# zhenyuw16/Uni3DETR

Hardware: AMD Instinct MI355X
Metric: scenes/sec (fwd+bwd) SUN-RGB-D 20k pts, 300 queries (higher is better)
Workload: dtype bf16

## Files before the change

include/u3d_hip.h:

```cpp
#ifndef U3D_HIP_H_
#define U3D_HIP_H_

#include <stddef.h>
#include <stdint.h>

#ifdef __cplusplus
extern "C" {
#endif

typedef struct ihipStream_t* u3d_stream;

enum {
  U3D_OK = 0,
  U3D_ERR_ARG = -1,
  U3D_ERR_UNSUPPORTED = -2,
  U3D_ERR_LAUNCH = -3,
  U3D_ERR_WORKSPACE = -4
};

enum { U3D_F32 = 0, U3D_BF16 = 1 };

int32_t u3d_version(void);
const char* u3d_strerror(int32_t code);

// ... 30 lines not shown

int32_t u3d_nbr_table(const u3d_bitgrid* target, const int32_t* q_coors, const int32_t* n_dev, int32_t n_cap,
                      const int32_t ksize[3], const int32_t stride[3], const int32_t pad[3], int32_t mode,
                      int32_t* nbr, int32_t ld, u3d_stream s);

int32_t u3d_nbr_table_k3(const u3d_bitgrid* target, const int32_t* q_coors, const int32_t* n_dev, int32_t n_cap,
                         const int32_t stride[3], const int32_t pad[3], int32_t mode, int32_t* nbr, int32_t ld, u3d_stream s);

int32_t u3d_dense_nbr_table(int32_t batch, const int32_t q_dims[3], const int32_t t_dims[3], const int32_t ksize[3],
                            const int32_t stride[3], const int32_t pad[3], int32_t mode, int32_t* nbr, int32_t ld,
                            u3d_stream s);

int64_t u3d_voxelize_hard_workspace(int32_t n_total, int32_t batch, int32_t max_pts_per_scene);
int32_t u3d_voxelize_hard(const float* points, const int32_t* scene_off, int32_t batch, int32_t n_total,
                          int32_t max_pts_per_scene, int32_t nfeat, const float voxel_size[3],
                          const float pc_range[6], int32_t max_points, int32_t max_voxels,
                          float* voxels, int32_t* coors, int32_t* num_points, float* mean,
                          int32_t* voxel_off, void* workspace, int64_t workspace_bytes, u3d_stream s);
int32_t u3d_voxelize_hard_chunked(const float* points, const int32_t* scene_off, int32_t batch, int32_t n_total,
                                  int32_t max_pts_per_scene, int32_t nfeat, const float voxel_size[3],
                                  const float pc_range[6], int32_t max_points, int32_t max_voxels,
                                  float* voxels, int32_t* coors, int32_t* num_points, float* mean,
                                  int32_t* voxel_off, void* workspace, int64_t workspace_bytes, u3d_stream s);

int32_t u3d_voxelize_dynamic(const float* points, const int32_t* scene_off, int32_t batch, int32_t n_total, int32_t nfeat,
                             const float voxel_size[3], const float pc_range[6], int32_t* coors, u3d_stream s);
int32_t u3d_scatter_mean(const float* points, const int32_t* rank, int32_t n_total, int32_t nfeat, float* sums,
                         int32_t* counts, int32_t n_voxels, u3d_stream s);

int32_t u3d_spconv_fwd(const void* in, const void* w, const int32_t* nbr, int32_t ld, void* out,
                       const int32_t* n_out_dev, int32_t n_out_cap, int32_t cin, int32_t cout, int32_t kvol,
                       int32_t transpose_w, int32_t dtype, u3d_stream s);

enum { U3D_FWD_EPI_PLAIN, U3D_FWD_EPI_ADD, U3D_FWD_EPI_STATS, U3D_FWD_EPI_AFFINE, U3D_FWD_EPI_COUNT };
enum { U3D_FWD_FAM_NONE, U3D_FWD_FAM_CONV_IN, U3D_FWD_FAM_DIRECT, U3D_FWD_FAM_GLDS, U3D_FWD_FAM_REG, U3D_FWD_FAM_COUNT };
typedef struct u3d_fwd_plan_info {
  int32_t family, kernel, rows, cols, partials, rows_per_partial, takes_addend;
} u3d_fwd_plan_info;
int32_t u3d_igemm_fwd_plan(int32_t n_out_cap, int32_t cin, int32_t cout, int32_t kvol, int32_t has_nbr, int32_t nmajor, int32_t epi,
                           u3d_fwd_plan_info* info);
int32_t u3d_igemm_fwd_bf16(const void* in, const void* w, const int32_t* nbr, int32_t ld, void* out,
                           const int32_t* n_out_dev, int32_t n_out_cap, int32_t cin, int32_t cout, int32_t kvol,
                           int32_t transpose_w, const void* addend, double* stats, u3d_stream s);
int32_t u3d_linear_bf16(const void* x, const void* w, const float* bias, int32_t relu, void* out, const int32_t* m_dev,
                        int32_t m_cap, int32_t k, int32_t n, u3d_stream s);
int64_t u3d_bn_fold_job_bytes(void);
int32_t u3d_bn_fold_job_blocks(int32_t kvol, int32_t cout, int32_t cin);
int32_t u3d_bn_fold_batched(const void* jobs, int32_t njobs, int32_t total_blocks, u3d_stream s);
int32_t u3d_igemm_fwd_affine_bf16(const void* in, const void* w_folded, const int32_t* nbr, int32_t ld, const float* shift, int32_t relu,
                                  void* out, const int32_t* n_out_dev, int32_t n_out_cap, int32_t cin, int32_t cout, int32_t kvol,
                                  u3d_stream s);
int32_t u3d_igemm_fwd_split_bf16(const void* in, const void* w, const int32_t* nbr, int32_t ld, float* out, const int32_t* n_out_dev,
                                 int32_t n_out_cap, int32_t cin, int32_t cout, int32_t kvol3, double* stats, const float* addend, u3d_stream s);
int32_t u3d_igemm_direct_split_bf16(const void* in, const void* w3, const int32_t* nbr, int32_t ld, float* out, const int32_t* n_out_dev,
                                    int32_t n_out_cap, int32_t n_in_cap, int32_t cin, int32_t cout, u3d_stream s);
int32_t u3d_igemm_direct_affine_bf16(const void* in, const void* w_folded, const int32_t* nbr, int32_t ld, const float* shift,
                                     int32_t relu, const void* addend, void* out, const int32_t* n_out_dev, int32_t n_out_cap,
                                     int32_t cin, int32_t cout, u3d_stream s);
int32_t u3d_split3_weights(const float* src, int64_t sk, int64_t sa, int64_t sb, int32_t k, int32_t a, int32_t b, void* dst, u3d_stream s);
typedef struct U3dSplitRowsJobs {
  const float* src[32];
  void* dst[32];
  int32_t ld[32], rows[32], cols[32];
  int32_t first_block[33];
  int32_t njobs;
} U3dSplitRowsJobs;
int32_t u3d_split_rows_batch(const U3dSplitRowsJobs* jobs, u3d_stream s);
int32_t u3d_sum3_f32(const float* a, const float* b, const float* c, float* out, int64_t n, u3d_stream s);
int64_t u3d_split3_job_bytes(void);
int32_t u3d_split3_job_blocks(int32_t k, int32_t a, int32_t b);
int32_t u3d_split3_weights_batch(const void* jobs, int32_t njobs, int32_t total_blocks, u3d_stream s);
int32_t u3d_split_rows_f32(const float* x, const int32_t* n_dev, int32_t n_cap, int32_t c, void* dst, u3d_stream s);
int32_t u3d_subm_halo_sizes(int32_t n_cap, int64_t* tile_rows_elems, int64_t* loc_elems, int32_t* tiles);
int32_t u3d_subm_halo_build(const int32_t* nbr, int32_t ld, const int32_t* n_dev, int32_t n_cap, int32_t* tile_rows,
                            uint16_t* loc, int32_t* tile_cnt, int32_t kvol, u3d_stream s);
int32_t u3d_subm_halo_wpack(const void* w_nmajor, void* w_packed, u3d_stream s);
int32_t u3d_subm_halo_wpack_batched(const void* const* srcs_dev, void* const* dsts_dev, int32_t n, u3d_stream s);
int32_t u3d_subm_halo_conv64_bf16(const void* in, const void* w_packed, const int32_t* tile_rows, const uint16_t* loc,
                                  const int32_t* tile_cnt, const int32_t* n_dev, int32_t n_cap, int32_t krev,
                                  const void* addend, void* out, double* stats, int32_t max_slots, u3d_stream s);
int32_t u3d_subm_halo_wpack128(const void* w_nmajor, void* w_packed, int32_t kvol, u3d_stream s);
int32_t u3d_subm_halo_wpack128_batched(const void* const* srcs_dev, void* const* dsts_dev, int32_t n, int32_t kvol, u3d_stream s);
int32_t u3d_subm_halo_conv128_bf16(const void* in, const void* w_packed, const int32_t* tile_rows, const uint16_t* loc,
                                   const int32_t* tile_cnt, const int32_t* n_dev, int32_t n_cap, int32_t krev,
                                   const void* addend, void* out, double* stats, int32_t max_slots, int32_t kvol, u3d_stream s);
int32_t u3d_subm_halo_conv64_affine_bf16(const void* in, const void* w_packed, const int32_t* tile_rows, const uint16_t* loc,
                                         const int32_t* tile_cnt, const int32_t* n_dev, int32_t n_cap, const void* addend, void* out,
                                         const float* shift, int32_t relu, int32_t max_slots, u3d_stream s);
int32_t u3d_subm_halo_conv128_affine_bf16(const void* in, const void* w_packed, const int32_t* tile_rows, const uint16_t* loc,
                                          const int32_t* tile_cnt, const int32_t* n_dev, int32_t n_cap, const void* addend, void* out,
                                          const float* shift, int32_t relu, int32_t max_slots, int32_t kvol, u3d_stream s);
int64_t u3d_subm_halo_wgrad64_workspace(void);
int32_t u3d_subm_halo_wgrad64_bf16(const void* x, const void* dy, const int32_t* tile_rows, const uint16_t* loc,
                                   const int32_t* tile_cnt, const int32_t* n_dev, int32_t n_cap, float* dw, void* workspace,
                                   int64_t workspace_bytes, int32_t max_slots, u3d_stream s);
int64_t u3d_igemm_wgrad_bf16_workspace(int32_t n_out_cap, int32_t cin, int32_t cout, int32_t kvol);
int32_t u3d_igemm_wgrad_bf16(const void* in, const void* dout, const int32_t* nbr, int32_t ld, float* dw,
                             const int32_t* n_out_dev, int32_t n_out_cap, int32_t cin, int32_t cout, int32_t kvol,
                             int32_t out_layout, void* workspace, int64_t workspace_bytes, u3d_stream s);
int32_t u3d_igemm_wgrad_plan(int32_t n_out_cap, int32_t cin, int32_t cout, int32_t kvol, int32_t has_nbr, int32_t out_layout,
                             int32_t* kernel, int32_t* tile, int32_t* nsplit, int64_t* workspace);

int64_t u3d_spconv_wgrad_workspace(int32_t n_out_cap, int32_t cin, int32_t cout, int32_t kvol);
int32_t u3d_spconv_wgrad(const void* in, const void* dout, const int32_t* nbr, int32_t ld, float* dw,
                         const int32_t* n_out_dev, int32_t n_out_cap, int32_t cin, int32_t cout, int32_t kvol,
                         int32_t dtype, void* workspace, int64_t workspace_bytes, u3d_stream s);

int64_t u3d_colsum_workspace(int32_t n, int32_t c);
int32_t u3d_colsum(const void* x, int32_t n, int32_t c, int32_t dtype, float* out, void* workspace,
                   int64_t workspace_bytes, u3d_stream s);

int64_t u3d_wgrad_batched_workspace(int32_t count, int32_t n_rows, int32_t cin, int32_t cout);
int32_t u3d_wgrad_batched_bf16(const void* const* in, const void* const* dout, float* const* dw, int32_t count,
                               const int32_t* n_dev, int32_t n_rows, int32_t cin, int32_t cout, void* workspace,
                               int64_t workspace_bytes, u3d_stream s);
int64_t u3d_colsum_batched_workspace(int32_t count, int32_t n, int32_t c);
int32_t u3d_colsum_batched(const void* const* x, float* const* out, int32_t count, int32_t n, int32_t c, int32_t dtype,
                           void* workspace, int64_t workspace_bytes, u3d_stream s);

int32_t u3d_skinny_wgrad_chunks(int32_t m);
int32_t u3d_skinny_wgrad_bf16(const void* dy, const void* x, int32_t m, int32_t n, int32_t k, float* partial, u3d_stream s);
int32_t u3d_skinny_wgrad_batched(const void* const* dy, const void* const* x, float* const* partial, const int32_t* n, const int32_t* k,
                                 int32_t count, int32_t m, int32_t dy_skinny, u3d_stream s);

int64_t u3d_bn_stats_workspace(int32_t n_cap, int32_t c);
int32_t u3d_bn_stats(const void* x, const int32_t* n_dev, int32_t n_cap, int32_t c, int32_t dtype,
                     double* sums, void* workspace, int64_t workspace_bytes, u3d_stream s);
int32_t u3d_bn_finalize(const double* sums, const int32_t* n_dev, int32_t n_cap, int32_t c, float eps, float momentum,
                        float* running_mean, float* running_var, int64_t* num_batches, float* mean, float* invstd,
                        u3d_stream s);
int32_t u3d_bn_forward_stats(const void* x, const int32_t* n_dev, int32_t n_cap, int32_t c, int32_t dtype, float eps,
                             float momentum, float* running_mean, float* running_var, int64_t* num_batches, float* mean,
                             float* invstd, void* workspace, int64_t workspace_bytes, u3d_stream s);
int32_t u3d_bn_finalize_partials(const double* partial, int32_t nblocks, int32_t rows_per_block, const int32_t* n_dev,
                                 int32_t n_cap, int32_t c, float eps, float momentum, float* running_mean, float* running_var,
                                 int64_t* num_batches, float* mean, float* invstd, u3d_stream s);
int32_t u3d_bn_apply(const void* x, const float* mean, const float* invstd, const float* gamma,
                     const float* beta, const void* residual, int32_t relu, void* y,
                     const int32_t* n_dev, int32_t n_cap, int32_t c, int32_t dtype, const int32_t* row_map, const void* post_add,
                     u3d_stream s);
int32_t u3d_bn_bwd_stats(const void* dy, const void* y, const void* x, const float* mean, const float* invstd,
                         const float* gamma, const float* beta, int32_t relu, const int32_t* n_dev, int32_t n_cap,
                         int32_t c, int32_t dtype, double* sums, void* workspace, int64_t workspace_bytes,
                         const int32_t* row_map, float* sums_f32, u3d_stream s);
int32_t u3d_bn_bwd_apply(const void* dy, const void* y, const void* x, const float* mean, const float* invstd,
                         const float* gamma, const float* beta, const double* sums, int32_t relu, void* dx, void* dres,
                         const int32_t* n_dev, int32_t n_cap, int32_t c, int32_t dtype, const int32_t* row_map, u3d_stream s);
int32_t u3d_bn_apply_planes(const float* x, const float* mean, const float* invstd, const float* gamma, const float* beta,
                            const float* residual, int32_t relu, float* y, void* planes, const int32_t* n_dev, int32_t n_cap,
                            int32_t c, const int32_t* row_map, const float* post_add, u3d_stream s);
int32_t u3d_bn_bwd_apply_planes(const float* dy, const float* y, const float* x, const float* mean, const float* invstd,
                                const float* gamma, const float* beta, const double* sums, int32_t relu, float* dx, float* dres,
                                void* planes, const int32_t* n_dev, int32_t n_cap, int32_t c, const int32_t* row_map, u3d_stream s);

int32_t u3d_to_dense(const void* feat, const int32_t* coors, const int32_t* n_dev, int32_t n_cap, int32_t c,
                     void* dense, int32_t dz, int32_t dy, int32_t dx, int32_t dtype, u3d_stream s);
int32_t u3d_from_dense(const void* dense, const int32_t* coors, const int32_t* n_dev, int32_t n_cap, int32_t c,
                       void* feat, int32_t dz, int32_t dy, int32_t dx, int32_t dtype, u3d_stream s);

int32_t u3d_gather_rows(const void* in, const int32_t* idx, int32_t n, int32_t row_bytes, void* out, u3d_stream s);
int32_t u3d_scatter_rows(const void* in, const int32_t* idx, int32_t n, int32_t row_bytes, void* out, u3d_stream s);

int32_t u3d_fps(const float* base, const int64_t* set_off, const int32_t* set_n, int32_t nsets, int32_t max_n,
                int32_t m, int32_t* out_idx, float* temp, int64_t temp_stride, int32_t* err, int64_t poll_ticks, int32_t max_wg,
                u3d_stream s);
int32_t u3d_fps2(const float* base, const float* base2, int32_t split, const int64_t* set_off, const int32_t* set_n,
                 int32_t nsets, int32_t max_n, int32_t m, int32_t* out_idx, float* temp, int64_t temp_stride, int32_t* err,
                 int64_t poll_ticks, int32_t max_wg, u3d_stream s);
int32_t u3d_fps_prep(const int32_t* coors, int32_t v_rows, const int32_t* scene_off, const int32_t* voxel_off, int32_t batch,
                     int32_t nfeat, float* vox, int64_t* set_off, int32_t* set_n, u3d_stream s);
int32_t u3d_fps_points(const float* pts, int32_t nfeat, const float* vox, const int32_t* idx, const int32_t* scene_off,
                       const int32_t* voxel_off, int32_t batch, int32_t m, float* out, u3d_stream s);
int32_t u3d_query_embed_fwd(const float* tgt, const float* anchor, const float* fps, const float* rnd, int32_t batch, int32_t nq,
                            int32_t groups, int32_t c, float* query_embeds, float* query, float* ref, float* ref_sig, u3d_stream s);
int32_t u3d_query_embed_bwd(const float* d_query_embeds, const float* d_query, const float* d_ref, const float* d_ref_sig,
                            const float* anchor, int32_t batch, int32_t nq, int32_t groups, int32_t c, float* d_tgt, float* d_anchor,
                            u3d_stream s);

int32_t u3d_match_cost(const float* cls, const float* box, const float* gt, const int32_t* labels,
                       const int32_t* gt_off, int32_t nlayers, int32_t batch, int32_t nq_total, int32_t ncls,
                       int32_t code_size, int32_t gmax, float w_cls, float w_reg, float w_iou, float alpha,
                       float gamma, float* cost, u3d_stream s);
int32_t u3d_lsa(const float* cost, const int32_t* gt_off, int32_t nlayers, int32_t batch, int32_t nq_total,
                int32_t nq, int32_t gmax, int32_t* assigned, u3d_stream s);

int32_t u3d_trilinear_fwd(const void* value, const float* grid, int32_t batch, int32_t nq, int32_t dz, int32_t dy, int32_t dx,
                          int32_t c, void* out, int32_t dtype, u3d_stream s);
int32_t u3d_trilinear_bwd(const void* value, const float* grid, const void* dout, int32_t batch, int32_t nq, int32_t dz,
                          int32_t dy, int32_t dx, int32_t c, float* dvalue, float* dgrid, int32_t dtype, u3d_stream s);

int32_t u3d_iou3d_rotated_aligned(const float* a, const float* b, int32_t n, float* out, u3d_stream s);

int64_t u3d_nms3d_workspace(int32_t n);
int32_t u3d_nms3d(const float* boxes, const int32_t* labels, int32_t n, float thr, uint8_t* keep, void* workspace,
                  int64_t workspace_bytes, u3d_stream s);

#define U3D_DET_TAIL_NONE 0
#define U3D_DET_TAIL_NMS 1
#define U3D_DET_TAIL_DECODE 2
#define U3D_DET_TAIL_MAX_K 8192
#define U3D_DET_TAIL_LDS_CAP 2048
int64_t u3d_det_tail_workspace(int32_t batch, int32_t nq, int32_t num_classes, int32_t max_num, int32_t box_dim);
int32_t u3d_det_tail(const float* prob, const float* fused, const float* boxes, int32_t batch, int32_t nq, int32_t num_classes,
                     int32_t box_dim, int32_t max_num, const float* center_range, float score_threshold, int32_t mode, float nms_thr,
                     const float* score_thr, int32_t num_thr, float* out_boxes, float* out_scores, int32_t* out_labels,
                     int32_t* out_count, int32_t* out_off, void* workspace, int64_t workspace_bytes, u3d_stream s);

#define U3D_DET_TAIL_SOFT_NMS 3
#define U3D_DET_TAIL_MERGE 4
int64_t u3d_det_tail_pp_workspace(int32_t batch, int32_t nq, int32_t num_classes, int32_t max_num, int32_t box_dim, int32_t mode);
int32_t u3d_det_tail_pp(const float* prob, const float* fused, const float* boxes, int32_t batch, int32_t nq, int32_t num_classes,
                        int32_t box_dim, int32_t max_num, const float* center_range, float score_threshold, int32_t mode, float nms_thr,
                        const float* score_thr, int32_t num_thr, float soft_sigma, float soft_prune, float* out_boxes, float* out_scores,
                        int32_t* out_labels, int32_t* out_count, int32_t* out_off, void* workspace, int64_t workspace_bytes, u3d_stream s);

int32_t u3d_tap_gather_sum(const void* p, const int32_t* nbr, int32_t ld, const int32_t* n_dev, int32_t n_cap, int32_t c,
                           int32_t kvol, int32_t dtype, void* out, u3d_stream s);
int32_t u3d_tap_gather_sum_add(const void* p, const int32_t* nbr, int32_t ld, const int32_t* n_dev, int32_t n_cap, int32_t c,
                               int32_t kvol, int32_t dtype, const void* addend, void* out, u3d_stream s);

int32_t u3d_layernorm_blocks(int32_t n);
int32_t u3d_layernorm_fwd(const void* x, int32_t x_dtype, int32_t n, int32_t c, const float* gamma, const float* beta,
                          float eps, int32_t relu, void* y, int32_t y_dtype, float* mean, float* rstd, u3d_stream s);
int32_t u3d_layernorm_bwd(const void* dy, int32_t y_dtype, const void* x, int32_t x_dtype, int32_t n, int32_t c,
                          const float* gamma, const float* beta, const float* mean, const float* rstd, int32_t relu,
                          void* dx, float* partial, u3d_stream s);

int64_t u3d_det_loss_workspace(int32_t L, int32_t m);
int32_t u3d_det_loss_fwd(const float* cls, const float* box, const float* iou_logit, const float* tgt, const int64_t* lab,
                         const float* w, const float* iou_true, const float* cls_avg, const float* npos, const float* code_w,
                         int32_t L, int32_t m, int32_t c, int32_t code, int32_t tdim, float alpha, float w_cls, float w_box,
                         float w_iou, float eps, float* out, void* workspace, int64_t workspace_bytes, u3d_stream s);
int32_t u3d_det_loss_bwd(const float* cls, const float* box, const float* iou_logit, const float* tgt, const int64_t* lab,
                         const float* w, const float* iou_true, const float* cls_avg, const float* npos, const float* code_w,
                         const float* gout, int32_t L, int32_t m, int32_t c, int32_t code, int32_t tdim, float alpha, float w_cls,
                         float w_box, float w_iou, float eps, float* dcls, float* dbox, float* diou, u3d_stream s);
int32_t u3d_loss_targets(const int32_t* asg, const float* gt, const int32_t* labels, const int32_t* gt_off, int32_t L, int32_t B,
                         int32_t Q, int32_t gd, int32_t ncls, int64_t* asg64, float* w, float* tgt, int64_t* lab, float* num_pos,
                         u3d_stream s);
int32_t u3d_denormalize_boxes(const float* codes, int32_t n, int32_t code, float* boxes, u3d_stream s);
int32_t u3d_box_decode_fwd(const void* tmp, int32_t dtype, const float* ref, int32_t n, int32_t code, const float* pc_range,
                           float eps, float* out, u3d_stream s);
int32_t u3d_box_decode_bwd(const void* tmp, int32_t dtype, const float* ref, const float* dout, int32_t n, int32_t code,
                           const float* pc_range, float eps, void* dtmp, float* dref, u3d_stream s);
int32_t u3d_refine_decode_fwd(const float* tmp, const float* ref_in, const float* ref_s, int32_t n, int32_t code,
                              const float* pc_range, float eps, float* out, float* ref_out, float* ref_sig, u3d_stream s);
int32_t u3d_sine_embed_fwd(const float* logits, const float* dim_t, int32_t n, int32_t nc, int32_t nfeat, int32_t out_dtype,
                           void* out, u3d_stream s);
int32_t u3d_sine_embed_bwd(const float* logits, const float* dim_t, const void* dout, int32_t dout_dtype, int32_t n, int32_t nc,
                           int32_t nfeat, float* dlogits, u3d_stream s);

int64_t u3d_adamw_workspace(int64_t n);
int32_t u3d_adamw_set_hyper(float* state, float lr, float beta1, float beta2, float eps, float weight_decay, float max_norm,
                            u3d_stream s);
int32_t u3d_adamw_step_state(float* param, const float* grad, float* exp_avg, float* exp_avg_sq, int64_t n, float* state,
                             const uint8_t* skip, void* workspace, int64_t workspace_bytes, u3d_stream s);
int32_t u3d_adamw_step_hold(float* param, const float* grad, float* exp_avg, float* exp_avg_sq, int64_t n, float* state,
                            const uint8_t* skip, const float* hold, void* workspace, int64_t workspace_bytes, u3d_stream s);
int32_t u3d_adamw_step_accum(float* param, const float* grad, float* acc, float* exp_avg, float* exp_avg_sq, float* ema, int64_t n,
                             float* state, float* acc_state, const uint8_t* skip, const float* hold, void* workspace,
                             int64_t workspace_bytes, u3d_stream s);
int32_t u3d_adamw_set_accum(float* acc_state, int32_t accum_steps, float ema_decay, u3d_stream s);
int32_t u3d_capacity_flag(const int32_t* const* counts, const int32_t* caps, int32_t n, float* flag, u3d_stream s);
int32_t u3d_adamw_step(float* param, const float* grad, float* exp_avg, float* exp_avg_sq, int64_t n, float lr, float beta1,
                       float beta2, float eps, float weight_decay, float max_norm, float* state, void* workspace,
                       int64_t workspace_bytes, u3d_stream s);

typedef struct u3d_permute_desc {
  int64_t src_off, dst_off;
  int32_t n, rows, cols, reserved;
  int64_t stride_k, stride_r, stride_c;
} u3d_permute_desc;
int32_t u3d_cast_bf16(const float* src, void* dst, int64_t n, u3d_stream s);
int32_t u3d_permute_block_elems(void);
int32_t u3d_permute_bf16_batched(const void* src, void* dst, const u3d_permute_desc* descs_dev, const int32_t* blocks_dev,
                                 int32_t nblocks, u3d_stream s);
int32_t u3d_permute_bf16_tiled(const void* src, void* dst, const u3d_permute_desc* descs_dev, const int32_t* tiles_dev,
                               int32_t ntiles, int32_t max_k, u3d_stream s);

int32_t u3d_soft_nms(const float* boxes, const float* scores, const int32_t* labels, int32_t n, int32_t num_classes, float sigma,
                     float prune, int32_t* out_idx, float* out_score, int32_t* out_cnt, u3d_stream s);
int64_t u3d_box_merge_workspace(int32_t n);
int32_t u3d_box_merge(const float* boxes, const int32_t* labels, int32_t n, float thr, float* merged, uint8_t* keep, void* workspace,
                      int64_t workspace_bytes, u3d_stream s);

int32_t u3d_eval_iou_argmax(const float* det_boxes, const float* det_scores, const int32_t* det_labels, const int32_t* det_off,
                            const float* gt_boxes, const int32_t* gt_labels, const int32_t* gt_off, int32_t n_scene, int32_t n_det,
                            float* iou_max, int32_t* jmax, int64_t* sort_key, u3d_stream s);
int32_t u3d_eval_segments(const int64_t* sorted_key, int32_t n_det, const int32_t* gt_labels, int32_t n_gt, int32_t num_classes,
                          int32_t* seg, int32_t* npos, u3d_stream s);
int32_t u3d_eval_first_hit(const int64_t* perm, int32_t n_det, const float* iou_max, const int32_t* jmax, const float* thr, int32_t n_thr,
                           int32_t n_gt, int32_t* first, u3d_stream s);
int32_t u3d_eval_tp(const int64_t* perm, int32_t n_det, const float* iou_max, const int32_t* jmax, const float* thr, int32_t n_thr,
                    int32_t n_gt, const int32_t* first, uint8_t* tp, u3d_stream s);
int32_t u3d_eval_ap(const uint8_t* tp, int32_t n_det, const int32_t* seg, const int32_t* npos, int32_t num_classes, int32_t n_thr,
                    int32_t n_gt, double* prec_ws, float* ap, double* rec, u3d_stream s);

int32_t u3d_kitti_convert(const float* boxes, const float* scores, const int32_t* labels, const int32_t* off, int32_t n_scene, int32_t n,
                          const float* calib, const float* img, const int32_t* label_code, int32_t n_label, const float* lim, float* rec,
                          int32_t* valid, u3d_stream s);
int32_t u3d_kitti_compact(const float* rec, const int32_t* valid, const int32_t* pos, int32_t n, float* out, u3d_stream s);
int32_t u3d_kitti_overlaps(const float* dt, const int32_t* dt_off, const float* gt, const int32_t* gt_off, const int64_t* ov_off,
                           int32_t n_scene, int64_t n_pairs, float* ov, u3d_stream s);
int32_t u3d_kitti_flags(const float* dt, const int32_t* dt_off, int32_t n_scene, int32_t n_dt, const float* gt, const int32_t* gt_off,
                        int32_t n_gt, const int32_t* cls, int32_t K, int8_t* gt_flag, int32_t* nvalid, int8_t* dt_flag, float* dc_iof,
                        u3d_stream s);
// ... 199 lines not shown
```

uni3detr_amd/csrc/rowops.hip:

```cpp
#include "common.h"
#include <type_traits>

typedef unsigned short u16;
__device__ __forceinline__ float ld_elem(const float* p, long long i) { return p[i]; }
__device__ __forceinline__ float ld_elem(const u16* p, long long i) { return __uint_as_float(((unsigned)p[i]) << 16); }
__device__ __forceinline__ void st_elem(float* p, long long i, float v) { p[i] = v; }
__device__ __forceinline__ void st_elem(u16* p, long long i, float v) {
  unsigned u = __float_as_uint(v);
  if ((u & 0x7fffffffu) > 0x7f800000u) { p[i] = (u16)((u >> 16) | 0x40u); return; }
  u += 0x7fffu + ((u >> 16) & 1u);
  p[i] = (u16)(u >> 16);
}

static inline int st_rows_per_block(int n_cap, int c) {
  if (n_cap >= 131072) return c >= 128 ? 256 : 512;
  return n_cap >= 32768 ? 128 : 16;
}

template <typename T> struct VecOf;
template <> struct VecOf<float> { static constexpr int N = 4; };
template <> struct VecOf<u16> { static constexpr int N = 8; };

template <typename T>
__device__ __forceinline__ void load_vec(const T* p, float* out);
template <>
__device__ __forceinline__ void load_vec<float>(const float* p, float* out) {
  float4 v = *(const float4*)p;
  out[0] = v.x; out[1] = v.y; out[2] = v.z; out[3] = v.w;
}
template <>
__device__ __forceinline__ void load_vec<u16>(const u16* p, float* out) {
  uint4 v = *(const uint4*)p;
  unsigned w[4] = {v.x, v.y, v.z, v.w};
#pragma unroll
  for (int i = 0; i < 4; ++i) { out[2 * i] = __uint_as_float(w[i] << 16); out[2 * i + 1] = __uint_as_float(w[i] & 0xffff0000u); }
}

static inline bool al16(const void* p) { return ((uintptr_t)p & 15) == 0; }
template <int V>
__device__ __forceinline__ void load_cols(const float* __restrict__ p, int col0, float* out) {
#pragma unroll
  for (int i = 0; i < V; i += 4) {
    const float4 t = *(const float4*)(p + col0 + i);
    out[i] = t.x; out[i + 1] = t.y; out[i + 2] = t.z; out[i + 3] = t.w;
  }
}
template <int V>
__device__ __forceinline__ void load_cols_d(const double* __restrict__ p, int col0, float scale, float* out) {
#pragma unroll
  for (int i = 0; i < V; i += 2) {
    const double2 t = *(const double2*)(p + col0 + i);
    out[i] = (float)t.x * scale; out[i + 1] = (float)t.y * scale;
  }
}

template <typename T, int MODE>
__global__ __launch_bounds__(256) void k_col_stats_vec(const T* __restrict__ x, const T* __restrict__ dy, const T* __restrict__ y,
                                                       const float* __restrict__ mean, const float* __restrict__ invstd,
                                                       const float* __restrict__ gamma, const float* __restrict__ beta, int relu,
                                                       const int* __restrict__ n_dev, int n_cap, int c, double* __restrict__ partial,
                                                       const int* __restrict__ row_map, int rows_per_block) {
  constexpr int V = VecOf<T>::N;
  extern __shared__ __attribute__((aligned(16))) char smem_raw[];
  double* red = (double*)smem_raw;
  const int n = min(*n_dev, n_cap);
  const int cv = c / V;
  const int cw = cv < 256 ? cv : 256;
  const int rl = 256 / cw;
  const int tcol = threadIdx.x % cw, trow = threadIdx.x / cw;
  const int r0 = blockIdx.x * rows_per_block;
  const int r1 = min(n, r0 + rows_per_block);
  for (int cb = 0; cb < cv; cb += cw) {
    const int vc = cb + tcol;
    float s0[V], s1[V];
#pragma unroll
    for (int e = 0; e < V; ++e) { s0[e] = 0.f; s1[e] = 0.f; }
    const bool active = vc < cv && trow < rl;
    if (active) {
      float mu[V], is[V], ga[V], be[V];
      const bool remask = MODE == 1 && relu && y == nullptr;
      if (MODE == 1) {
        load_cols<V>(mean, vc * V, mu);
        load_cols<V>(invstd, vc * V, is);
        if (remask) { load_cols<V>(gamma, vc * V, ga); load_cols<V>(beta, vc * V, be); }
      }
#pragma unroll 4
      for (int r = r0 + trow; r < r1; r += rl) {
        const long long o = (long long)r * c + (long long)vc * V;
        float xv[V];
        load_vec<T>(x + o, xv);
        if (MODE == 0) {
#pragma unroll
          for (int e = 0; e < V; ++e) { s0[e] += xv[e]; s1[e] += xv[e] * xv[e]; }
        } else {
          float gv[V], yv[V];
          const long long oy = row_map ? (long long)row_map[r] * c + (long long)vc * V : o;
          load_vec<T>(dy + oy, gv);
          if (relu && !remask) load_vec<T>(y + oy, yv);
#pragma unroll
          for (int e = 0; e < V; ++e) {
            float g = gv[e];
            if (remask) yv[e] = (xv[e] - mu[e]) * is[e] * ga[e] + be[e];
            if (relu && !(yv[e] > 0.f)) g = 0.f;
            s0[e] += g;
            s1[e] += g * ((xv[e] - mu[e]) * is[e]);
          }
        }
      }
    }
    const int ncol = cw * V;
    if (trow < rl) {
#pragma unroll
      for (int e = 0; e < V; ++e) {
        red[(0 * rl + trow) * ncol + tcol * V + e] = (double)s0[e];
        red[(1 * rl + trow) * ncol + tcol * V + e] = (double)s1[e];
      }
    }
    __syncthreads();
    const int NP = rl >= 32 ? 8 : 1;
    if (NP > 1) {
      double* red2 = red + 2 * rl * ncol;
      for (int i = threadIdx.x; i < 2 * ncol * NP; i += 256) {
        const int o = i % (2 * ncol), pp = i / (2 * ncol), which = o / ncol, col = o % ncol;
        double a = 0.0;
        for (int j = pp; j < rl; j += NP) a += red[(which * rl + j) * ncol + col];
        red2[pp * 2 * ncol + o] = a;
      }
      __syncthreads();
      for (int i = threadIdx.x; i < 2 * ncol; i += 256) {
        const int which = i / ncol, col = i % ncol;
        if (cb * V + col < c) {
          double a = 0.0;
          for (int pp = 0; pp < NP; ++pp) a += red2[pp * 2 * ncol + i];
          partial[((long long)blockIdx.x * 2 + which) * c + cb * V + col] = a;
        }
      }
    } else {
      for (int i = threadIdx.x; i < 2 * ncol; i += 256) {
        int which = i / ncol, col = i % ncol;
        if (cb * V + col < c) {
          double a = 0.0;
          for (int j = 0; j < rl; ++j) a += red[(which * rl + j) * ncol + col];
          partial[((long long)blockIdx.x * 2 + which) * c + cb * V + col] = a;
        }
      }
    }
    __syncthreads();
  }
}

template <typename T, int MODE>
__global__ __launch_bounds__(256) void k_col_stats(const T* __restrict__ x, const T* __restrict__ dy, const T* __restrict__ y,
                                                   const float* __restrict__ mean, const float* __restrict__ invstd,
                                                   const float* __restrict__ gamma, const float* __restrict__ beta, int relu,
                                                   const int* __restrict__ n_dev, int n_cap, int c, double* __restrict__ partial,
                                                   int rows_per_block) {
  __shared__ double red[2][256];
  const int n = min(*n_dev, n_cap);
  const int cw = c < 256 ? c : 256;
  const int rl = 256 / cw;
  const int tcol = threadIdx.x % cw, trow = threadIdx.x / cw;
  const int r0 = blockIdx.x * rows_per_block;
  const int r1 = min(n, r0 + rows_per_block);
  for (int cb = 0; cb < c; cb += cw) {
    int col = cb + tcol;
    double s0 = 0.0, s1 = 0.0;
    if (col < c && trow < rl) {
      float mu = 0.f, is = 0.f, ga = 0.f, be = 0.f;
      const bool remask = MODE == 1 && relu && y == nullptr;
      if (MODE == 1) { mu = mean[col]; is = invstd[col]; }
      if (remask) { ga = gamma[col]; be = beta[col]; }
      for (int r = r0 + trow; r < r1; r += rl) {
        long long o = (long long)r * c + col;
        if (MODE == 0) {
          float v = ld_elem(x, o);
          s0 += (double)v;
          s1 += (double)v * (double)v;
        } else {
          float g = ld_elem(dy, o);
          float yv = remask ? (ld_elem(x, o) - mu) * is * ga + be : (relu ? ld_elem(y, o) : 1.f);
          if (relu && !(yv > 0.f)) g = 0.f;
          float xh = (ld_elem(x, o) - mu) * is;
          s0 += (double)g;
          s1 += (double)g * (double)xh;
        }
      }
    }
    red[0][threadIdx.x] = s0;
    red[1][threadIdx.x] = s1;
    __syncthreads();
    if (trow == 0 && col < c) {
      double a0 = 0.0, a1 = 0.0;
      for (int j = 0; j < rl; ++j) { a0 += red[0][j * cw + tcol]; a1 += red[1][j * cw + tcol]; }
      partial[((long long)blockIdx.x * 2 + 0) * c + col] = a0;
      partial[((long long)blockIdx.x * 2 + 1) * c + col] = a1;
    }
    __syncthreads();
  }
}

#define FIN_THREADS 1024
#define FIN_LANES (FIN_THREADS / 16)
__device__ __forceinline__ void fin_reduce(const double* __restrict__ partial, int used, int c, int col0, double (*red)[16]) {
  const int v = threadIdx.x & 15, bl = threadIdx.x >> 4;
  const int which = v >> 3, col = col0 + (v & 7);
  double a = 0.0;
  if (col < c) {
#pragma unroll 8
    for (int b = bl; b < used; b += FIN_LANES) a += partial[((long long)b * 2 + which) * c + col];
  }
  red[bl][v] = a;
  __syncthreads();
  if (threadIdx.x < 16) {
    double s0 = 0.0, s1 = 0.0, s2 = 0.0, s3 = 0.0;
#pragma unroll 4
    for (int j = 0; j < FIN_LANES; j += 4) { s0 += red[j][threadIdx.x]; s1 += red[j + 1][threadIdx.x]; s2 += red[j + 2][threadIdx.x]; s3 += red[j + 3][threadIdx.x]; }
    red[0][threadIdx.x] = (s0 + s1) + (s2 + s3);
  }
  __syncthreads();
}

__global__ __launch_bounds__(FIN_THREADS) void k_col_stats_final(const double* __restrict__ partial, int nblocks, const int* __restrict__ n_dev,
                                                                 int n_cap, int c, double* __restrict__ sums, float* __restrict__ sums_f32,
                                                                 int rows_per_block) {
  __shared__ double red[FIN_LANES][16];
  const int n = min(*n_dev, n_cap);
  int used = rows_per_block > 0 ? (n + rows_per_block - 1) / rows_per_block : nblocks;
  if (used > nblocks) used = nblocks;
  const int col0 = blockIdx.x * 8;
  fin_reduce(partial, used, c, col0, red);
  if (threadIdx.x < 16) {
    const int which = threadIdx.x >> 3, col = col0 + (threadIdx.x & 7);
    if (col < c) {
      const double s = red[0][threadIdx.x];
      sums[which * c + col] = s;
      if (sums_f32) sums_f32[which * c + col] = (float)s;
    }
  }
}

extern "C" int64_t u3d_bn_stats_workspace(int32_t n_cap, int32_t c) {
  return (int64_t)u3d_cdiv(n_cap > 0 ? n_cap : 1, st_rows_per_block(n_cap, c)) * 2 * c * 8;
}

template <int MODE>
static int run_stats(const void* x, const void* dy, const void* y, const float* mean, const float* invstd, const float* gamma,
                     const float* beta, int relu, const int32_t* n_dev, int n_cap, int c, int dtype, double* sums, void* ws, int64_t ws_bytes, hipStream_t s,
                     const int32_t* row_map = nullptr, float* sums_f32 = nullptr) {
  U3D_REQUIRE(x && n_dev && sums && ws && c > 0, U3D_ERR_ARG);
  U3D_REQUIRE(!row_map || (dtype == U3D_F32 ? c % 4 == 0 : c % 8 == 0), U3D_ERR_UNSUPPORTED);
  if (n_cap <= 0) { hipMemsetAsync(sums, 0, sizeof(double) * 2 * c, s); return U3D_OK; }
  U3D_REQUIRE(ws_bytes >= u3d_bn_stats_workspace(n_cap, c), U3D_ERR_WORKSPACE);
  const int rpb = st_rows_per_block(n_cap, c);
  int nb = u3d_cdiv(n_cap, rpb);
  const bool pal = al16(mean) && al16(invstd) && al16(gamma) && al16(beta);
  U3D_REQUIRE(!row_map || pal, U3D_ERR_ARG);
  if (dtype == U3D_F32) {
    if (c % 4 == 0 && pal) {
      int cw = (c / 4) < 256 ? (c / 4) : 256; int rl = 256 / cw;
      size_t lds = (size_t)2 * (rl + (rl >= 32 ? 8 : 0)) * cw * 4 * sizeof(double);
      hipLaunchKernelGGL((k_col_stats_vec<float, MODE>), dim3(nb), dim3(256), lds, s, (const float*)x, (const float*)dy, (const float*)y, mean, invstd, gamma, beta, relu, n_dev, n_cap, c, (double*)ws, row_map, rpb);
    } else {
      hipLaunchKernelGGL((k_col_stats<float, MODE>), dim3(nb), dim3(256), 0, s, (const float*)x, (const float*)dy, (const float*)y, mean, invstd, gamma, beta, relu, n_dev, n_cap, c, (double*)ws, rpb);
    }
  } else if (dtype == U3D_BF16) {
    if (c % 8 == 0 && pal) {
      int cw = (c / 8) < 256 ? (c / 8) : 256; int rl = 256 / cw;
      size_t lds = (size_t)2 * (rl + (rl >= 32 ? 8 : 0)) * cw * 8 * sizeof(double);
      hipLaunchKernelGGL((k_col_stats_vec<u16, MODE>), dim3(nb), dim3(256), lds, s, (const u16*)x, (const u16*)dy, (const u16*)y, mean, invstd, gamma, beta, relu, n_dev, n_cap, c, (double*)ws, row_map, rpb);
    } else {
      hipLaunchKernelGGL((k_col_stats<u16, MODE>), dim3(nb), dim3(256), 0, s, (const u16*)x, (const u16*)dy, (const u16*)y, mean, invstd, gamma, beta, relu, n_dev, n_cap, c, (double*)ws, rpb);
    }
  } else return U3D_ERR_UNSUPPORTED;
  hipLaunchKernelGGL(k_col_stats_final, dim3(u3d_cdiv(c, 8)), dim3(FIN_THREADS), 0, s, (const double*)ws, nb, n_dev, n_cap, c, sums, sums_f32, rpb);
  U3D_CHECK_LAUNCH();
  return U3D_OK;
}

extern "C" int32_t u3d_bn_stats(const void* x, const int32_t* n_dev, int32_t n_cap, int32_t c, int32_t dtype, double* sums,
                                void* workspace, int64_t workspace_bytes, u3d_stream s) {
  return run_stats<0>(x, nullptr, nullptr, nullptr, nullptr, nullptr, nullptr, 0, n_dev, n_cap, c, dtype, sums, workspace, workspace_bytes, s);
}
extern "C" int32_t u3d_bn_bwd_stats(const void* dy, const void* y, const void* x, const float* mean, const float* invstd,
                                    const float* gamma, const float* beta, int32_t relu, const int32_t* n_dev, int32_t n_cap,
                                    int32_t c, int32_t dtype, double* sums, void* workspace, int64_t workspace_bytes,
                                    const int32_t* row_map, float* sums_f32, u3d_stream s) {
  U3D_REQUIRE(dy && mean && invstd && (!relu || y || (gamma && beta)), U3D_ERR_ARG);
  return run_stats<1>(x, dy, y, mean, invstd, gamma, beta, relu, n_dev, n_cap, c, dtype, sums, workspace, workspace_bytes, s, row_map, sums_f32);
}

#define CS_ROWS 32
template <typename T, int V>
__global__ __launch_bounds__(256) void k_colsum_partial(const T* __restrict__ x, int n, int c, float* __restrict__ partial) {
  __shared__ float red[256 * 8];
  const int cv = (c + V - 1) / V;
  const int cw = cv < 256 ? cv : 256;
  const int rl = 256 / cw;
  const int tcol = threadIdx.x % cw, trow = threadIdx.x / cw;
  const int r0 = blockIdx.x * CS_ROWS, r1 = min(n, r0 + CS_ROWS);
  for (int cb = 0; cb < cv; cb += cw) {
    const int vc = cb + tcol;
    float s[V];
#pragma unroll
    for (int e = 0; e < V; ++e) s[e] = 0.f;
    if (vc < cv && trow < rl) {
      for (int r = r0 + trow; r < r1; r += rl) {
        const long long o = (long long)r * c + (long long)vc * V;
        float xv[V];
        if constexpr (V == 1) xv[0] = ld_elem(x, o); else load_vec<T>(x + o, xv);
#pragma unroll
        for (int e = 0; e < V; ++e) s[e] += xv[e];
      }
    }
    if (trow < rl) {
#pragma unroll
      for (int e = 0; e < V; ++e) red[(trow * cw + tcol) * V + e] = s[e];
    }
    __syncthreads();
    for (int i = threadIdx.x; i < cw * V; i += 256) {
      if (cb * V + i < c) {
        float a = 0.f;
        for (int j = 0; j < rl; ++j) a += red[j * cw * V + i];
        partial[(long long)blockIdx.x * c + cb * V + i] = a;
      }
    }
    __syncthreads();
  }
}
__global__ __launch_bounds__(256) void k_colsum_final(const float* __restrict__ partial, int nb, int c, float* __restrict__ out) {
  int col = blockIdx.x * 4 + (threadIdx.x >> 6), lane = threadIdx.x & 63;
  if (col >= c) return;
  float s = 0.f;
  for (int b = lane; b < nb; b += 64) s += partial[(long long)b * c + col];
  s = u3d_wave_sum(s);
  if (lane == 0) out[col] = s;
}
#define U3D_COLSUM_BATCH_MAX 64
struct ColsumBatch { const void* x[U3D_COLSUM_BATCH_MAX]; float* out[U3D_COLSUM_BATCH_MAX]; };
struct ColsumGroups { unsigned char mult[U3D_COLSUM_BATCH_MAX]; };
template <typename T, int V>
__global__ __launch_bounds__(256) void k_colsum_partial_b(ColsumBatch bt, int n, int c, float* __restrict__ partial, long long pstride) {
  const T* x = (const T*)bt.x[blockIdx.y];
  partial += (long long)blockIdx.y * pstride;
  __shared__ float red[256 * 8];
  const int cv = (c + V - 1) / V;
  const int cw = cv < 256 ? cv : 256;
  const int rl = 256 / cw;
  const int tcol = threadIdx.x % cw, trow = threadIdx.x / cw;
  const int r0 = blockIdx.x * CS_ROWS, r1 = min(n, r0 + CS_ROWS);
  for (int cb = 0; cb < cv; cb += cw) {
    const int vc = cb + tcol;
    float s[V];
#pragma unroll
    for (int e = 0; e < V; ++e) s[e] = 0.f;
    if (vc < cv && trow < rl) {
      for (int r = r0 + trow; r < r1; r += rl) {
        const long long o = (long long)r * c + (long long)vc * V;
        float xv[V];
        if constexpr (V == 1) xv[0] = ld_elem(x, o); else load_vec<T>(x + o, xv);
#pragma unroll
        for (int e = 0; e < V; ++e) s[e] += xv[e];
      }
    }
    if (trow < rl) {
#pragma unroll
      for (int e = 0; e < V; ++e) red[(trow * cw + tcol) * V + e] = s[e];
    }
    __syncthreads();
    for (int i = threadIdx.x; i < cw * V; i += 256) {
      if (cb * V + i < c) {
        float a = 0.f;
        for (int j = 0; j < rl; ++j) a += red[j * cw * V + i];
        partial[(long long)blockIdx.x * c + cb * V + i] = a;
      }
    }
    __syncthreads();
  }
}
__global__ __launch_bounds__(256) void k_colsum_final_b(ColsumBatch bt, ColsumGroups gr, const float* __restrict__ partial, int nb, int c,
                                                        long long pstride) {
  int col = blockIdx.x * 4 + (threadIdx.x >> 6), lane = threadIdx.x & 63;
  const int g = gr.mult[blockIdx.y];
  if (col >= c || g == 0) return;
  const float* p = partial + (long long)blockIdx.y * pstride;
  nb *= g;
  float s = 0.f;
  for (int b = lane; b < nb; b += 64) s += p[(long long)b * c + col];
  s = u3d_wave_sum(s);
  if (lane == 0) bt.out[blockIdx.y][col] = s;
}
extern "C" int64_t u3d_colsum_batched_workspace(int32_t count, int32_t n, int32_t c) {
  return (int64_t)count * u3d_cdiv(n > 0 ? n : 1, CS_ROWS) * c * 4;
}
extern "C" int32_t u3d_colsum_batched(const void* const* x, float* const* out, int32_t count, int32_t n, int32_t c, int32_t dtype,
                                      void* workspace, int64_t workspace_bytes, u3d_stream s) {
  U3D_REQUIRE(x && out && workspace && count >= 0 && count <= U3D_COLSUM_BATCH_MAX && n > 0 && c > 0, U3D_ERR_ARG);
  if (count == 0) return U3D_OK;
  U3D_REQUIRE(workspace_bytes >= u3d_colsum_batched_workspace(count, n, c), U3D_ERR_WORKSPACE);
  ColsumBatch bt;
  for (int i = 0; i < U3D_COLSUM_BATCH_MAX; ++i) { bt.x[i] = i < count ? x[i] : nullptr; bt.out[i] = i < count ? out[i] : nullptr; }
  const int nb = u3d_cdiv(n, CS_ROWS);
  const long long pstride = (long long)nb * c;
  float* ws = (float*)workspace;
  dim3 grid(nb, count);
  if (dtype == U3D_F32) {
    if (c % 4 == 0) hipLaunchKernelGGL((k_colsum_partial_b<float, 4>), grid, dim3(256), 0, s, bt, n, c, ws, pstride);
    else hipLaunchKernelGGL((k_colsum_partial_b<float, 1>), grid, dim3(256), 0, s, bt, n, c, ws, pstride);
  } else if (dtype == U3D_BF16) {
    if (c % 8 == 0) hipLaunchKernelGGL((k_colsum_partial_b<u16, 8>), grid, dim3(256), 0, s, bt, n, c, ws, pstride);
    else hipLaunchKernelGGL((k_colsum_partial_b<u16, 1>), grid, dim3(256), 0, s, bt, n, c, ws, pstride);
  } else return U3D_ERR_UNSUPPORTED;
  ColsumGroups gr;
  for (int i = 0; i < U3D_COLSUM_BATCH_MAX; ++i) gr.mult[i] = 0;
  for (int i = 0, lead = 0; i < count; ++i) {
    if (i > 0 && out[i] == out[i - 1]) { gr.mult[lead]++; } else { lead = i; gr.mult[i] = 1; }
  }
  hipLaunchKernelGGL(k_colsum_final_b, dim3(u3d_cdiv(c, 4), count), dim3(256), 0, s, bt, gr, (const float*)ws, nb, c, pstride);
  U3D_CHECK_LAUNCH();
  return U3D_OK;
}

extern "C" int64_t u3d_colsum_workspace(int32_t n, int32_t c) { return (int64_t)u3d_cdiv(n > 0 ? n : 1, CS_ROWS) * c * 4; }
extern "C" int32_t u3d_colsum(const void* x, int32_t n, int32_t c, int32_t dtype, float* out, void* workspace,
                              int64_t workspace_bytes, u3d_stream s) {
  U3D_REQUIRE(out && c > 0 && n >= 0, U3D_ERR_ARG);
  if (n == 0) { hipMemsetAsync(out, 0, sizeof(float) * c, s); return U3D_OK; }
  U3D_REQUIRE(x && workspace && workspace_bytes >= u3d_colsum_workspace(n, c), U3D_ERR_WORKSPACE);
  const int nb = u3d_cdiv(n, CS_ROWS);
  float* ws = (float*)workspace;
  if (dtype == U3D_F32) {
    if (c % 4 == 0) hipLaunchKernelGGL((k_colsum_partial<float, 4>), dim3(nb), dim3(256), 0, s, (const float*)x, n, c, ws);
    else hipLaunchKernelGGL((k_colsum_partial<float, 1>), dim3(nb), dim3(256), 0, s, (const float*)x, n, c, ws);
  } else if (dtype == U3D_BF16) {
    if (c % 8 == 0) hipLaunchKernelGGL((k_colsum_partial<u16, 8>), dim3(nb), dim3(256), 0, s, (const u16*)x, n, c, ws);
    else hipLaunchKernelGGL((k_colsum_partial<u16, 1>), dim3(nb), dim3(256), 0, s, (const u16*)x, n, c, ws);
  } else return U3D_ERR_UNSUPPORTED;
  hipLaunchKernelGGL(k_colsum_final, dim3(u3d_cdiv(c, 4)), dim3(256), 0, s, (const float*)ws, nb, c, out);
  U3D_CHECK_LAUNCH();
  return U3D_OK;
}

__global__ void k_bn_finalize(const double* __restrict__ sums, const int* __restrict__ n_dev, int n_cap, int c, float eps,
                              float momentum, float* __restrict__ running_mean, float* __restrict__ running_var,
                              long long* __restrict__ num_batches, float* __restrict__ mean, float* __restrict__ invstd) {
  int i = blockIdx.x * blockDim.x + threadIdx.x;
  int n = min(*n_dev, n_cap);
  if (i == 0 && num_batches) *num_batches += 1;
  if (i >= c) return;
  double nn = n > 0 ? (double)n : 1.0;
  double mu = sums[i] / nn;
  double var = sums[c + i] / nn - mu * mu;
  if (var < 0.0) var = 0.0;
  mean[i] = (float)mu;
  invstd[i] = (float)(1.0 / sqrt(var + (double)eps));
  if (running_mean) {
    double unbiased = n > 1 ? var * nn / (nn - 1.0) : var;
    running_mean[i] = (1.f - momentum) * running_mean[i] + momentum * (float)mu;
    running_var[i] = (1.f - momentum) * running_var[i] + momentum * (float)unbiased;
  }
}

extern "C" int32_t u3d_bn_finalize(const double* sums, const int32_t* n_dev, int32_t n_cap, int32_t c, float eps,
                                   float momentum, float* running_mean, float* running_var, int64_t* num_batches,
                                   float* mean, float* invstd, u3d_stream s) {
  U3D_REQUIRE(sums && n_dev && mean && invstd && c > 0 && (!running_mean || running_var), U3D_ERR_ARG);
  hipLaunchKernelGGL(k_bn_finalize, dim3(u3d_cdiv(c, 256)), dim3(256), 0, s, sums, n_dev, n_cap, c, eps, momentum,
                     running_mean, running_var, (long long*)num_batches, mean, invstd);
  U3D_CHECK_LAUNCH();
  return U3D_OK;
}

template <typename T>
__global__ void k_bn_apply(const T* __restrict__ x, const float* __restrict__ mean, const float* __restrict__ invstd,
                           const float* __restrict__ gamma, const float* __restrict__ beta, const T* __restrict__ res, int relu,
                           T* __restrict__ y, const int* __restrict__ n_dev, int n_cap, int c) {
  long long total = (long long)min(*n_dev, n_cap) * c;
  for (long long i = (long long)blockIdx.x * blockDim.x + threadIdx.x; i < total; i += (long long)gridDim.x * blockDim.x) {
    int col = (int)(i % c);
    float v = (ld_elem(x, i) - mean[col]) * invstd[col] * gamma[col] + beta[col];
    if (res) v += ld_elem(res, i);
    if (relu) v = v > 0.f ? v : 0.f;
    st_elem(y, i, v);
  }
}

template <typename T>
__global__ void k_bn_bwd_apply(const T* __restrict__ dy, const T* __restrict__ y, const T* __restrict__ x,
                               const float* __restrict__ mean, const float* __restrict__ invstd, const float* __restrict__ gamma,
                               const float* __restrict__ beta, const double* __restrict__ sums, int relu, T* __restrict__ dx,
                               T* __restrict__ dres, const int* __restrict__ n_dev, int n_cap, int c) {
  int n = min(*n_dev, n_cap);
  long long total = (long long)n * c;
  float inv_n = n > 0 ? 1.f / (float)n : 0.f;
  for (long long i = (long long)blockIdx.x * blockDim.x + threadIdx.x; i < total; i += (long long)gridDim.x * blockDim.x) {
    int col = (int)(i % c);
    float g = ld_elem(dy, i);
    if (relu) {
      float yv = y ? ld_elem(y, i) : (ld_elem(x, i) - mean[col]) * invstd[col] * gamma[col] + beta[col];
      if (!(yv > 0.f)) g = 0.f;
    }
    float is = invstd[col];
    float xh = (ld_elem(x, i) - mean[col]) * is;
    float mg = (float)sums[col] * inv_n, mgx = (float)sums[c + col] * inv_n;
    st_elem(dx, i, gamma[col] * is * (g - mg - xh * mgx));
    if (dres) st_elem(dres, i, g);
  }
}

__global__ __launch_bounds__(FIN_THREADS) void k_bn_final_finalize(const double* __restrict__ partial, int nblocks, int rows_per_block,
                                                                   const int* __restrict__ n_dev,
                                                                   int n_cap, int c, float eps, float momentum, float* __restrict__ running_mean,
                                                                   float* __restrict__ running_var, long long* __restrict__ num_batches,
                                                                   float* __restrict__ mean, float* __restrict__ invstd) {
  __shared__ double red[FIN_LANES][16];
  if (blockIdx.x == 0 && threadIdx.x == 0 && num_batches) *num_batches += 1;
  const int n = min(*n_dev, n_cap);
  int used = rows_per_block > 0 ? (n + rows_per_block - 1) / rows_per_block : nblocks;
  if (used > nblocks) used = nblocks;
  const int col0 = blockIdx.x * 8;
  fin_reduce(partial, used, c, col0, red);
  const int col = col0 + threadIdx.x;
  if (threadIdx.x >= 8 || col >= c) return;
  const double s0 = red[0][threadIdx.x], s1 = red[0][8 + threadIdx.x];
  const double nn = n > 0 ? (double)n : 1.0;
  const double mu = s0 / nn;
  double var = s1 / nn - mu * mu;
  if (var < 0.0) var = 0.0;
  mean[col] = (float)mu;
  invstd[col] = (float)(1.0 / sqrt(var + (double)eps));
  if (running_mean) {
    const double unbiased = n > 1 ? var * nn / (nn - 1.0) : var;
    running_mean[col] = (1.f - momentum) * running_mean[col] + momentum * (float)mu;
    running_var[col] = (1.f - momentum) * running_var[col] + momentum * (float)unbiased;
  }
}
extern "C" int32_t u3d_bn_forward_stats(const void* x, const int32_t* n_dev, int32_t n_cap, int32_t c, int32_t dtype, float eps,
                                        float momentum, float* running_mean, float* running_var, int64_t* num_batches, float* mean,
                                        float* invstd, void* workspace, int64_t workspace_bytes, u3d_stream s) {
  U3D_REQUIRE(x && n_dev && mean && invstd && workspace && c > 0 && (!running_mean || running_var), U3D_ERR_ARG);
  U3D_REQUIRE(workspace_bytes >= u3d_bn_stats_workspace(n_cap, c), U3D_ERR_WORKSPACE);
  const int rpb = st_rows_per_block(n_cap, c);
  const int nb = n_cap > 0 ? u3d_cdiv(n_cap, rpb) : 0;
  if (nb > 0) {
    const bool f32 = dtype == U3D_F32;
    if (!f32 && dtype != U3D_BF16) return U3D_ERR_UNSUPPORTED;
    const int v = f32 ? 4 : 8;
    if (c % v == 0) {
      int cw = (c / v) < 256 ? (c / v) : 256; int rl = 256 / cw;
      size_t lds = (size_t)2 * (rl + (rl >= 32 ? 8 : 0)) * cw * v * sizeof(double);
      if (f32) hipLaunchKernelGGL((k_col_stats_vec<float, 0>), dim3(nb), dim3(256), lds, s, (const float*)x, nullptr, nullptr, nullptr, nullptr, nullptr, nullptr, 0, n_dev, n_cap, c, (double*)workspace, (const int*)nullptr, rpb);
      else hipLaunchKernelGGL((k_col_stats_vec<u16, 0>), dim3(nb), dim3(256), lds, s, (const u16*)x, nullptr, nullptr, nullptr, nullptr, nullptr, nullptr, 0, n_dev, n_cap, c, (double*)workspace, (const int*)nullptr, rpb);
    } else {
      if (f32) hipLaunchKernelGGL((k_col_stats<float, 0>), dim3(nb), dim3(256), 0, s, (const float*)x, nullptr, nullptr, nullptr, nullptr, nullptr, nullptr, 0, n_dev, n_cap, c, (double*)workspace, rpb);
      else hipLaunchKernelGGL((k_col_stats<u16, 0>), dim3(nb), dim3(256), 0, s, (const u16*)x, nullptr, nullptr, nullptr, nullptr, nullptr, nullptr, 0, n_dev, n_cap, c, (double*)workspace, rpb);
    }
  }
  hipLaunchKernelGGL(k_bn_final_finalize, dim3(u3d_cdiv(c, 8)), dim3(FIN_THREADS), 0, s, (const double*)workspace, nb, rpb, n_dev, n_cap, c,
                     eps, momentum, running_mean, running_var, (long long*)num_batches, mean, invstd);
  U3D_CHECK_LAUNCH();
  return U3D_OK;
}
extern "C" int32_t u3d_bn_finalize_partials(const double* partial, int32_t nblocks, int32_t rows_per_block, const int32_t* n_dev,
                                            int32_t n_cap, int32_t c, float eps, float momentum, float* running_mean,
                                            float* running_var, int64_t* num_batches, float* mean, float* invstd, u3d_stream s) {
  U3D_REQUIRE(partial && n_dev && mean && invstd && c > 0 && nblocks >= 0 && rows_per_block >= 0 && (!running_mean || running_var), U3D_ERR_ARG);
  hipLaunchKernelGGL(k_bn_final_finalize, dim3(u3d_cdiv(c, 8)), dim3(FIN_THREADS), 0, s, partial, nblocks, rows_per_block, n_dev, n_cap, c, eps, momentum,
                     running_mean, running_var, (long long*)num_batches, mean, invstd);
  U3D_CHECK_LAUNCH();
  return U3D_OK;
}

template <typename T>
__device__ __forceinline__ void store_vec(T* p, const float* v);
template <>
__device__ __forceinline__ void store_vec<float>(float* p, const float* v) { *(float4*)p = make_float4(v[0], v[1], v[2], v[3]); }
template <>
__device__ __forceinline__ void store_vec<u16>(u16* p, const float* v) {
  typedef float f32x8_t __attribute__((ext_vector_type(8)));
  typedef __bf16 bf16x8_t __attribute__((ext_vector_type(8)));
  f32x8_t f = {v[0], v[1], v[2], v[3], v[4], v[5], v[6], v[7]};
  *(bf16x8_t*)p = __builtin_convertvector(f, bf16x8_t);
}

__device__ __forceinline__ void store_planes4(u16* p, long long plane, const float* v) {
  typedef float f32x4_t __attribute__((ext_vector_type(4)));
  typedef __bf16 bf16x4_t __attribute__((ext_vector_type(4)));
  const f32x4_t f = {v[0], v[1], v[2], v[3]};
  const bf16x4_t h = __builtin_convertvector(f, bf16x4_t);
  const bf16x4_t l = __builtin_convertvector(f - __builtin_convertvector(h, f32x4_t), bf16x4_t);
  *(bf16x4_t*)p = h;
  *(bf16x4_t*)(p + plane) = l;
}
template <typename T, bool PLANES = false>
__global__ __launch_bounds__(256) void k_bn_apply_vec(const T* __restrict__ x, const float* __restrict__ mean, const float* __restrict__ invstd,
                                                      const float* __restrict__ gamma, const float* __restrict__ beta,
                                                      const T* __restrict__ res, int relu, T* __restrict__ y,
                                                      const int* __restrict__ n_dev, int n_cap, int c, const int* __restrict__ row_map,
                                                      const T* __restrict__ post_add, u16* __restrict__ planes = nullptr) {
  constexpr int V = VecOf<T>::N;
  static_assert(!PLANES || V == 4, "planes are an f32 feature");
  const int n = min(*n_dev, n_cap), cv = c / V, rpb = 256 / cv;
  const int vc = threadIdx.x % cv, rl = threadIdx.x / cv;
  float mu[V], is[V], ga[V], be[V];
  load_cols<V>(mean, vc * V, mu); load_cols<V>(invstd, vc * V, is); load_cols<V>(gamma, vc * V, ga); load_cols<V>(beta, vc * V, be);
  for (int r = blockIdx.x * rpb + rl; r < n; r += gridDim.x * rpb) {
    const long long o = (long long)r * c + (long long)vc * V;
    float xv[V], rv[V], out[V];
    load_vec<T>(x + o, xv);
    if (res) load_vec<T>(res + o, rv);
#pragma unroll
    for (int e = 0; e < V; ++e) {
      float v = (xv[e] - mu[e]) * is[e] * ga[e] + be[e];
      if (res) v += rv[e];
      if (relu) v = v > 0.f ? v : 0.f;
      out[e] = v;
    }
    const long long oy = row_map ? (long long)row_map[r] * c + (long long)vc * V : o;
    if (post_add) {
      float pv[V];
      load_vec<T>(post_add + oy, pv);
#pragma unroll
      for (int e = 0; e < V; ++e) out[e] += pv[e];
    }
    store_vec<T>(y + oy, out);
    if constexpr (PLANES) store_planes4(planes + oy, (long long)n_cap * c, out);
  }
  if constexpr (PLANES) {
    const float z[4] = {0.f, 0.f, 0.f, 0.f};
    for (int r = n + blockIdx.x * rpb + rl; r < n_cap; r += gridDim.x * rpb)
      store_planes4(planes + (long long)r * c + (long long)vc * V, (long long)n_cap * c, z);
  }
}

template <typename T, bool PLANES = false>
__global__ __launch_bounds__(256) void k_bn_bwd_apply_vec(const T* __restrict__ dy, const T* __restrict__ y, const T* __restrict__ x,
                                                          const float* __restrict__ mean, const float* __restrict__ invstd,
                                                          const float* __restrict__ gamma, const float* __restrict__ beta,
                                                          const double* __restrict__ sums, int relu, T* __restrict__ dx,
                                                          T* __restrict__ dres, const int* __restrict__ n_dev, int n_cap, int c,
                                                          const int* __restrict__ row_map, u16* __restrict__ planes = nullptr) {
  constexpr int V = VecOf<T>::N;
  static_assert(!PLANES || V == 4, "planes are an f32 feature");
  const int n = min(*n_dev, n_cap), cv = c / V, rpb = 256 / cv;
  const int vc = threadIdx.x % cv, rl = threadIdx.x / cv;
  const float inv_n = n > 0 ? 1.f / (float)n : 0.f;
  const bool remask = relu && y == nullptr;
  float mu[V], is[V], ga[V], be[V], mg[V], mgx[V];
  load_cols<V>(mean, vc * V, mu); load_cols<V>(invstd, vc * V, is); load_cols<V>(gamma, vc * V, ga);
  if (remask) load_cols<V>(beta, vc * V, be);
  else {
#pragma unroll
    for (int e = 0; e < V; ++e) be[e] = 0.f;
  }
  load_cols_d<V>(sums, vc * V, inv_n, mg);
  load_cols_d<V>(sums + c, vc * V, inv_n, mgx);
#pragma unroll 2
  for (int r = blockIdx.x * rpb + rl; r < n; r += gridDim.x * rpb) {
    const long long o = (long long)r * c + (long long)vc * V;
    float gv[V], xv[V], yv[V], dxv[V];
    const long long oy = row_map ? (long long)row_map[r] * c + (long long)vc * V : o;
    load_vec<T>(dy + oy, gv);
    load_vec<T>(x + o, xv);
    if (relu && !remask) load_vec<T>(y + oy, yv);
#pragma unroll
    for (int e = 0; e < V; ++e) {
      float g = gv[e];
      if (remask) yv[e] = (xv[e] - mu[e]) * is[e] * ga[e] + be[e];
      if (relu && !(yv[e] > 0.f)) g = 0.f;
      const float xh = (xv[e] - mu[e]) * is[e];
      dxv[e] = ga[e] * is[e] * (g - mg[e] - xh * mgx[e]);
      gv[e] = g;
    }
    store_vec<T>(dx + o, dxv);
    if constexpr (PLANES) store_planes4(planes + o, (long long)n_cap * c, dxv);
    if (dres) store_vec<T>(dres + o, gv);
  }
  if constexpr (PLANES) {
    const float z[4] = {0.f, 0.f, 0.f, 0.f};
    for (int r = n + blockIdx.x * rpb + rl; r < n_cap; r += gridDim.x * rpb)
      store_planes4(planes + (long long)r * c + (long long)vc * V, (long long)n_cap * c, z);
  }
}

static inline bool bn_vec_ok(int c, int v) { return c % v == 0 && (c / v) <= 256 && 256 % (c / v) == 0; }
static inline int bn_vec_grid(int n_cap, int c, int v) {
  int rpb = 256 / (c / v);
  long long b = ((long long)n_cap + rpb - 1) / rpb;
  return (int)(b < 1 ? 1 : (b > 2048 ? 2048 : b));
}

static inline int ew_grid(long long total) {
  long long b = (total + 255) / 256;
  return (int)(b < 1 ? 1 : (b > 8192 ? 8192 : b));
}

extern "C" int32_t u3d_bn_apply(const void* x, const float* mean, const float* invstd, const float* gamma, const float* beta,
                                const void* residual, int32_t relu, void* y, const int32_t* n_dev, int32_t n_cap, int32_t c,
                                int32_t dtype, const int32_t* row_map, const void* post_add, u3d_stream s) {
  U3D_REQUIRE(x && mean && invstd && gamma && beta && y && n_dev && c > 0, U3D_ERR_ARG);
  U3D_REQUIRE(!row_map || (!residual && bn_vec_ok(c, dtype == U3D_F32 ? 4 : 8)), U3D_ERR_UNSUPPORTED);
  U3D_REQUIRE(!post_add || bn_vec_ok(c, dtype == U3D_F32 ? 4 : 8), U3D_ERR_UNSUPPORTED);
  const bool pal = al16(mean) && al16(invstd) && al16(gamma) && al16(beta);
  U3D_REQUIRE(!(row_map || post_add) || pal, U3D_ERR_ARG);
  if (n_cap <= 0) return U3D_OK;
  int g = ew_grid((long long)n_cap * c);
  if (dtype == U3D_F32 && bn_vec_ok(c, 4) && pal)
    hipLaunchKernelGGL(k_bn_apply_vec<float>, dim3(bn_vec_grid(n_cap, c, 4)), dim3(256), 0, s, (const float*)x, mean, invstd, gamma, beta, (const float*)residual, relu, (float*)y, n_dev, n_cap, c, row_map, (const float*)post_add);
  else if (dtype == U3D_BF16 && bn_vec_ok(c, 8) && pal)
    hipLaunchKernelGGL(k_bn_apply_vec<u16>, dim3(bn_vec_grid(n_cap, c, 8)), dim3(256), 0, s, (const u16*)x, mean, invstd, gamma, beta, (const u16*)residual, relu, (u16*)y, n_dev, n_cap, c, row_map, (const u16*)post_add);
  else if (dtype == U3D_F32)
    hipLaunchKernelGGL(k_bn_apply<float>, dim3(g), dim3(256), 0, s, (const float*)x, mean, invstd, gamma, beta, (const float*)residual, relu, (float*)y, n_dev, n_cap, c);
  else if (dtype == U3D_BF16)
    hipLaunchKernelGGL(k_bn_apply<u16>, dim3(g), dim3(256), 0, s, (const u16*)x, mean, invstd, gamma, beta, (const u16*)residual, relu, (u16*)y, n_dev, n_cap, c);
  else return U3D_ERR_UNSUPPORTED;
  U3D_CHECK_LAUNCH();
  return U3D_OK;
}

extern "C" int32_t u3d_bn_bwd_apply(const void* dy, const void* y, const void* x, const float* mean, const float* invstd,
                                    const float* gamma, const float* beta, const double* sums, int32_t relu, void* dx, void* dres,
                                    const int32_t* n_dev, int32_t n_cap, int32_t c, int32_t dtype, const int32_t* row_map, u3d_stream s) {
  U3D_REQUIRE(dy && x && mean && invstd && gamma && sums && dx && n_dev && c > 0 && (!relu || y || beta), U3D_ERR_ARG);
  U3D_REQUIRE(!row_map || (!dres && bn_vec_ok(c, dtype == U3D_F32 ? 4 : 8)), U3D_ERR_UNSUPPORTED);
  const bool pal = al16(mean) && al16(invstd) && al16(gamma) && al16(beta) && al16(sums);
  U3D_REQUIRE(!row_map || pal, U3D_ERR_ARG);
  if (n_cap <= 0) return U3D_OK;
  int g = ew_grid((long long)n_cap * c);
  if (dtype == U3D_F32 && bn_vec_ok(c, 4) && pal)
    hipLaunchKernelGGL(k_bn_bwd_apply_vec<float>, dim3(bn_vec_grid(n_cap, c, 4)), dim3(256), 0, s, (const float*)dy, (const float*)y, (const float*)x, mean, invstd, gamma, beta, sums, relu, (float*)dx, (float*)dres, n_dev, n_cap, c, row_map);
  else if (dtype == U3D_BF16 && bn_vec_ok(c, 8) && pal)
    hipLaunchKernelGGL(k_bn_bwd_apply_vec<u16>, dim3(bn_vec_grid(n_cap, c, 8)), dim3(256), 0, s, (const u16*)dy, (const u16*)y, (const u16*)x, mean, invstd, gamma, beta, sums, relu, (u16*)dx, (u16*)dres, n_dev, n_cap, c, row_map);
  else if (dtype == U3D_F32)
    hipLaunchKernelGGL(k_bn_bwd_apply<float>, dim3(g), dim3(256), 0, s, (const float*)dy, (const float*)y, (const float*)x, mean, invstd, gamma, beta, sums, relu, (float*)dx, (float*)dres, n_dev, n_cap, c);
  else if (dtype == U3D_BF16)
    hipLaunchKernelGGL(k_bn_bwd_apply<u16>, dim3(g), dim3(256), 0, s, (const u16*)dy, (const u16*)y, (const u16*)x, mean, invstd, gamma, beta, sums, relu, (u16*)dx, (u16*)dres, n_dev, n_cap, c);
  else return U3D_ERR_UNSUPPORTED;
  U3D_CHECK_LAUNCH();
  return U3D_OK;
}

extern "C" int32_t u3d_bn_apply_planes(const float* x, const float* mean, const float* invstd, const float* gamma, const float* beta,
                                       const float* residual, int32_t relu, float* y, void* planes, const int32_t* n_dev, int32_t n_cap,
                                       int32_t c, const int32_t* row_map, const float* post_add, u3d_stream s) {
  U3D_REQUIRE(x && mean && invstd && gamma && beta && y && planes && n_dev && c > 0, U3D_ERR_ARG);
  if (!bn_vec_ok(c, 4) || !(al16(mean) && al16(invstd) && al16(gamma) && al16(beta)) || (row_map && residual)) return U3D_ERR_UNSUPPORTED;
  if (n_cap <= 0) return U3D_OK;
  hipLaunchKernelGGL((k_bn_apply_vec<float, true>), dim3(bn_vec_grid(n_cap, c, 4)), dim3(256), 0, s, x, mean, invstd, gamma, beta, residual, relu, y,
                     n_dev, n_cap, c, row_map, post_add, (u16*)planes);
  U3D_CHECK_LAUNCH();
  return U3D_OK;
}
extern "C" int32_t u3d_bn_bwd_apply_planes(const float* dy, const float* y, const float* x, const float* mean, const float* invstd,
                                           const float* gamma, const float* beta, const double* sums, int32_t relu, float* dx, float* dres,
                                           void* planes, const int32_t* n_dev, int32_t n_cap, int32_t c, const int32_t* row_map, u3d_stream s) {
  U3D_REQUIRE(dy && x && mean && invstd && gamma && sums && dx && planes && n_dev && c > 0 && (!relu || y || beta), U3D_ERR_ARG);
  if (!bn_vec_ok(c, 4) || !(al16(mean) && al16(invstd) && al16(gamma) && al16(beta) && al16(sums)) || (row_map && dres)) return U3D_ERR_UNSUPPORTED;
  if (n_cap <= 0) return U3D_OK;
  hipLaunchKernelGGL((k_bn_bwd_apply_vec<float, true>), dim3(bn_vec_grid(n_cap, c, 4)), dim3(256), 0, s, dy, y, x, mean, invstd, gamma, beta, sums, relu,
                     dx, dres, n_dev, n_cap, c, row_map, (u16*)planes);
  U3D_CHECK_LAUNCH();
  return U3D_OK;
}

template <bool TO_DENSE>
__global__ void k_dense_rows(const uint32_t* __restrict__ src, const int4* __restrict__ coors, const int* __restrict__ n_dev,
                             int n_cap, int row_words, uint32_t* __restrict__ dst, int dz, int dy, int dx) {
  long long total = (long long)min(*n_dev, n_cap) * row_words;
  for (long long t = (long long)blockIdx.x * blockDim.x + threadIdx.x; t < total; t += (long long)gridDim.x * blockDim.x) {
    int r = (int)(t / row_words), w = (int)(t % row_words);
    int4 c = coors[r];
    long long cell = (((long long)c.x * dz + c.y) * dy + c.z) * dx + c.w;
    if (TO_DENSE) dst[cell * row_words + w] = src[t];
    else dst[t] = src[cell * row_words + w];
  }
}

static int run_dense(bool to_dense, const void* a, const int32_t* coors, const int32_t* n_dev, int n_cap, int c, void* b, int dz,
                     int dy, int dx, int dtype, hipStream_t s) {
  U3D_REQUIRE(a && coors && n_dev && b && c > 0, U3D_ERR_ARG);
  int row_bytes = c * (dtype == U3D_BF16 ? 2 : 4);
  U3D_REQUIRE((row_bytes & 3) == 0, U3D_ERR_UNSUPPORTED);
  if (n_cap <= 0) return U3D_OK;
  int rw = row_bytes / 4;
  int g = ew_grid((long long)n_cap * rw);
  if (to_dense) hipLaunchKernelGGL(k_dense_rows<true>, dim3(g), dim3(256), 0, s, (const uint32_t*)a, (const int4*)coors, n_dev, n_cap, rw, (uint32_t*)b, dz, dy, dx);
  else hipLaunchKernelGGL(k_dense_rows<false>, dim3(g), dim3(256), 0, s, (const uint32_t*)a, (const int4*)coors, n_dev, n_cap, rw, (uint32_t*)b, dz, dy, dx);
  U3D_CHECK_LAUNCH();
  return U3D_OK;
}

extern "C" int32_t u3d_to_dense(const void* feat, const int32_t* coors, const int32_t* n_dev, int32_t n_cap, int32_t c,
                                void* dense, int32_t dz, int32_t dy, int32_t dx, int32_t dtype, u3d_stream s) {
  return run_dense(true, feat, coors, n_dev, n_cap, c, dense, dz, dy, dx, dtype, s);
}
extern "C" int32_t u3d_from_dense(const void* dense, const int32_t* coors, const int32_t* n_dev, int32_t n_cap, int32_t c,
                                  void* feat, int32_t dz, int32_t dy, int32_t dx, int32_t dtype, u3d_stream s) {
  return run_dense(false, dense, coors, n_dev, n_cap, c, feat, dz, dy, dx, dtype, s);
}

template <typename T>
__global__ __launch_bounds__(256) void k_tap_gather_sum(const T* __restrict__ p, const int* __restrict__ nbr, int ld,
                                                        const int* __restrict__ n_dev, int n_cap, int c, int kvol, T* __restrict__ out,
                                                        const T* __restrict__ addend) {
  constexpr int V = VecOf<T>::N;
  const int n = min(*n_dev, n_cap), cv = c / V;
  const long long total = (long long)n * cv;
  const long long prow = (long long)kvol * c;
  for (long long t = (long long)blockIdx.x * 256 + threadIdx.x; t < total; t += (long long)gridDim.x * 256) {
    const int i = (int)(t / cv), vc = (int)(t % cv);
    float acc[V];
#pragma unroll
    for (int e = 0; e < V; ++e) acc[e] = 0.f;
    if (addend) load_vec<T>(addend + (long long)i * c + (long long)vc * V, acc);
    for (int k = 0; k < kvol; ++k) {
      const int o = nbr[(long long)k * ld + i];
      if (o >= 0) {
        float v[V];
        load_vec<T>(p + (long long)o * prow + (long long)k * c + (long long)vc * V, v);
#pragma unroll
        for (int e = 0; e < V; ++e) acc[e] += v[e];
      }
    }
    store_vec<T>(out + (long long)i * c + (long long)vc * V, acc);
  }
}
extern "C" int32_t u3d_tap_gather_sum(const void* p, const int32_t* nbr, int32_t ld, const int32_t* n_dev, int32_t n_cap, int32_t c,
                                      int32_t kvol, int32_t dtype, void* out, u3d_stream s) {
  return u3d_tap_gather_sum_add(p, nbr, ld, n_dev, n_cap, c, kvol, dtype, nullptr, out, s);
}
extern "C" int32_t u3d_tap_gather_sum_add(const void* p, const int32_t* nbr, int32_t ld, const int32_t* n_dev, int32_t n_cap, int32_t c,
                                          int32_t kvol, int32_t dtype, const void* addend, void* out, u3d_stream s) {
  U3D_REQUIRE(p && nbr && n_dev && out && c > 0 && kvol > 0, U3D_ERR_ARG);
  if (n_cap <= 0) return U3D_OK;
  if (dtype == U3D_BF16 && c % 8 == 0) {
    int g = ew_grid((long long)n_cap * (c / 8));
    hipLaunchKernelGGL(k_tap_gather_sum<u16>, dim3(g), dim3(256), 0, s, (const u16*)p, nbr, ld, n_dev, n_cap, c, kvol, (u16*)out, (const u16*)addend);
  } else if (dtype == U3D_F32 && c % 4 == 0) {
    int g = ew_grid((long long)n_cap * (c / 4));
    hipLaunchKernelGGL(k_tap_gather_sum<float>, dim3(g), dim3(256), 0, s, (const float*)p, nbr, ld, n_dev, n_cap, c, kvol, (float*)out, (const float*)addend);
  } else return U3D_ERR_UNSUPPORTED;
  U3D_CHECK_LAUNCH();
  return U3D_OK;
}


#define LN_ROWS_PER_BLOCK 8
#define LN_MAXJ 16

template <typename T, int NJ>
__device__ __forceinline__ void ln_load_row(const T* __restrict__ p, int c, int lane, float* v) {
  if constexpr (NJ == 4 && std::is_same<T, float>::value) {
    float4 t = *(const float4*)(p + lane * 4);
    v[0] = t.x; v[1] = t.y; v[2] = t.z; v[3] = t.w;
  } else if constexpr (NJ == 4) {
    uint2 t = *(const uint2*)(p + lane * 4);
    v[0] = __uint_as_float(t.x << 16); v[1] = __uint_as_float(t.x & 0xffff0000u);
    v[2] = __uint_as_float(t.y << 16); v[3] = __uint_as_float(t.y & 0xffff0000u);
  } else if constexpr (NJ > 0) {
#pragma unroll
    for (int j = 0; j < NJ; ++j) v[j] = ld_elem(p, lane * NJ + j);
  } else {
#pragma unroll
    for (int j = 0; j < LN_MAXJ; ++j) { const int col = lane + 64 * j; v[j] = col < c ? ld_elem(p, col) : 0.f; }
  }
}
template <typename T, int NJ>
__device__ __forceinline__ void ln_store_row(T* __restrict__ p, int c, int lane, const float* v) {
  if constexpr (NJ == 4 && std::is_same<T, float>::value) {
    *(float4*)(p + lane * 4) = make_float4(v[0], v[1], v[2], v[3]);
  } else if constexpr (NJ == 4) {
    typedef float f4 __attribute__((ext_vector_type(4)));
    typedef __bf16 b4 __attribute__((ext_vector_type(4)));
    f4 f = {v[0], v[1], v[2], v[3]};
    *(b4*)(p + lane * 4) = __builtin_convertvector(f, b4);
  } else if constexpr (NJ > 0) {
#pragma unroll
    for (int j = 0; j < NJ; ++j) st_elem(p, lane * NJ + j, v[j]);
  } else {
#pragma unroll
    for (int j = 0; j < LN_MAXJ; ++j) { const int col = lane + 64 * j; if (col < c) st_elem(p, col, v[j]); }
  }
}
template <int NJ>
__device__ __forceinline__ int ln_col(int lane, int j) { return NJ > 0 ? lane * NJ + j : lane + 64 * j; }

template <typename TX, typename TY, int NJ>
__global__ __launch_bounds__(256) void k_layernorm_fwd(const TX* __restrict__ x, int n, int c, const float* __restrict__ gamma,
                                                       const float* __restrict__ beta, float eps, int relu, TY* __restrict__ y,
                                                       float* __restrict__ mean, float* __restrict__ rstd) {
  constexpr int J = NJ > 0 ? NJ : LN_MAXJ;
  const int lane = threadIdx.x & 63, wv = threadIdx.x >> 6;
  float ga[J], be[J];
#pragma unroll
// ... 205 lines not shown
```

uni3detr_amd/native.py:

```python
import collections
import ctypes as C
import os

import numpy as np
import torch

from . import abi

_HERE = os.path.dirname(os.path.abspath(__file__))
LIB_PATH = os.environ.get("U3D_LIB_PATH") or os.path.join(_HERE, "libu3d_hip.so")

_ABI = abi.load()
_K = _ABI.constants


def _struct(c_name, py_name):
    return abi.structure(_ABI.structs[c_name], py_name)


def _slot_names(prefix):
    names = sorted((v, n[len(prefix):]) for n, v in _K.items() if n.startswith(prefix))
    assert [v for v, _ in names] == list(range(len(names))) and names[-1][1] == "COUNT" and _K[prefix + "COUNT"] == len(names) - 1
    return [n for _, n in names[:-1]]

# ... 746 lines not shown
        if layout is not None and layout[1]:
            stats = torch.empty((layout[0], 2, cout), dtype=torch.float64, device=xs.device)
            tr = layout[1]
    region = timed_begin()
    assert addend is None or (addend.dtype == torch.float32 and tuple(addend.shape) == (n_out, cout))
    _check(lib().u3d_igemm_fwd_split_bf16(_ptr(xs), _ptr(w3), _ptr(nbr3), nbr3.shape[1], _ptr(out), _ptr(n_out_dev), n_out, cin, cout, kvol3,
                                          _ptr(stats), _ptr(addend), _stream()), "igemm_fwd_split_bf16")
    if region is not None:
        timed_end(region, tag, xs.shape[0] // 2, n_out, cin, cout, kvol3 // 3, nbr3, split=True)
    return (out, stats, tr) if want_stats else out


WGRAD_KERNELS = ("none", "conv_in", "narrow", "glds8_256", "glds_256", "glds_128", "glds_64", "reg_32", "reg_16")


def igemm_wgrad_plan(n_out, cin, cout, kvol, has_nbr, out_oik=False):
    k, tile, ns, ws = C.c_int32(0), C.c_int32(0), C.c_int32(0), C.c_int64(0)
    if lib().u3d_igemm_wgrad_plan(n_out, cin, cout, kvol, int(bool(has_nbr)), 1 if out_oik else 0, C.byref(k), C.byref(tile), C.byref(ns),
                                  C.byref(ws)) != 0:
        return None
    return WGRAD_KERNELS[k.value], tile.value, ns.value, ws.value


def spconv_wgrad(inp, dout, nbr, n_out_dev, kvol, out_oik=False, out=None):
    cin, cout, n_out = inp.shape[1], dout.shape[1], dout.shape[0]
    bf16 = bool(inp.dtype == torch.bfloat16 and USE_IGEMM_V2)
    v2 = bf16 and cin % 16 == 0 and cout % 16 == 0
    assert v2 or not out_oik, "out_oik needs the bf16 implicit-GEMM weight-gradient path"
    shape = (cout, cin, kvol) if out_oik else (kvol, cin, cout)
    plan = igemm_wgrad_plan(n_out, cin, cout, kvol, nbr is not None, out_oik) if bf16 else None
    region = timed_begin()
    if plan is None and not v2:
        dw = spconv_wgrad_generic(inp, dout, nbr, n_out_dev, kvol)
    else:
        if out is not None and v2 and out.is_contiguous() and out.dtype == torch.float32 and out.numel() == kvol * cin * cout:
            dw = out.view(shape)
        else:
            dw = torch.empty(shape, dtype=torch.float32, device=inp.device)
        if plan is not None:
            ws = torch.empty(plan[3], dtype=torch.uint8, device=inp.device)
            _check(lib().u3d_igemm_wgrad_bf16(_ptr(inp), _ptr(dout), _ptr(nbr), nbr.shape[1] if nbr is not None else 0, _ptr(dw),
                                              _ptr(n_out_dev), n_out, cin, cout, kvol, 1 if out_oik else 0, _ptr(ws), plan[3], _stream()),
                   "igemm_wgrad_bf16")
        else:
            gen = spconv_wgrad_generic(inp, dout, nbr, n_out_dev, kvol)
            dw.copy_(gen.permute(2, 1, 0) if out_oik else gen)
    if region is not None:
        timed_end(region, "spconv_wgrad", inp.shape[0], n_out, cin, cout, kvol, nbr, act_bytes=inp.element_size(), w_bytes=4, v2=v2)
    return dw


def spconv_wgrad_generic(inp, dout, nbr, n_out_dev, kvol):
    cin, cout, n_out = inp.shape[1], dout.shape[1], dout.shape[0]
    dw = torch.empty((kvol, cin, cout), dtype=torch.float32, device=inp.device)
    wsb = int(lib().u3d_spconv_wgrad_workspace(n_out, cin, cout, kvol))
    ws = torch.empty(wsb, dtype=torch.uint8, device=inp.device)
    ld = nbr.shape[1] if nbr is not None else 0
    _check(lib().u3d_spconv_wgrad(_ptr(inp), _ptr(dout), _ptr(nbr), ld, _ptr(dw), _ptr(n_out_dev), n_out, cin, cout, kvol,
                                  dtype_code(inp), _ptr(ws), wsb, _stream()), "spconv_wgrad")
    return dw


def colsum(x):
    x = x if x.is_contiguous() else x.contiguous()
    n, c = x.shape
    out = torch.empty((c,), dtype=torch.float32, device=x.device)
    wsb = int(lib().u3d_colsum_workspace(n, c))
    ws = torch.empty(max(wsb, 4), dtype=torch.uint8, device=x.device)
    _check(lib().u3d_colsum(_ptr(x), n, c, dtype_code(x), _ptr(out), _ptr(ws), wsb, _stream()), "colsum")
    return out


def bn_stats(x, n_dev):
    n, c = x.shape
    sums = torch.empty((2, c), dtype=torch.float64, device=x.device)
    wsb = int(lib().u3d_bn_stats_workspace(n, c))
    ws = torch.empty(wsb, dtype=torch.uint8, device=x.device)
    _check(lib().u3d_bn_stats(_ptr(x), _ptr(n_dev), n, c, dtype_code(x), _ptr(sums), _ptr(ws), wsb, _stream()), "bn_stats")
    return sums


def bn_finalize(sums, n_dev, n_cap, eps, momentum, running_mean=None, running_var=None, num_batches=None):
    c = sums.shape[1]
    mean = torch.empty((c,), dtype=torch.float32, device=sums.device)
    invstd = torch.empty((c,), dtype=torch.float32, device=sums.device)
    _check(lib().u3d_bn_finalize(_ptr(sums), _ptr(n_dev), n_cap, c, eps, momentum, _ptr(running_mean), _ptr(running_var),
                                 _ptr(num_batches), _ptr(mean), _ptr(invstd), _stream()), "bn_finalize")
    return mean, invstd


def bn_forward_stats(x, n_dev, eps, momentum, running_mean=None, running_var=None, num_batches=None):
    n, c = x.shape
    mean = torch.empty((c,), dtype=torch.float32, device=x.device)
    invstd = torch.empty((c,), dtype=torch.float32, device=x.device)
    wsb = int(lib().u3d_bn_stats_workspace(n, c))
    ws = torch.empty(max(wsb, 16), dtype=torch.uint8, device=x.device)
    _check(lib().u3d_bn_forward_stats(_ptr(x), _ptr(n_dev), n, c, dtype_code(x), eps, momentum, _ptr(running_mean), _ptr(running_var),
                                      _ptr(num_batches), _ptr(mean), _ptr(invstd), _ptr(ws), ws.numel(), _stream()), "bn_forward_stats")
    return mean, invstd


def bn_apply(x, mean, invstd, gamma, beta, residual, relu, n_dev, row_map=None, post_add=None, want_planes=False):
    n, c = x.shape
    y = torch.empty_like(x)
    if want_planes:
        planes = None
        if x.dtype == torch.float32 and x.is_cuda:
            planes = torch.empty((2 * n, c), dtype=torch.bfloat16, device=x.device)
            rc = lib().u3d_bn_apply_planes(_ptr(x), _ptr(mean), _ptr(invstd), _ptr(gamma), _ptr(beta), _ptr(residual), int(relu), _ptr(y),
                                           _ptr(planes), _ptr(n_dev), n, c, _ptr(row_map), _ptr(post_add), _stream())
            if rc == 0:
                return y, planes
            if rc != U3D_ERR_UNSUPPORTED:
                _check(rc, "bn_apply_planes")
            planes = None
        _check(lib().u3d_bn_apply(_ptr(x), _ptr(mean), _ptr(invstd), _ptr(gamma), _ptr(beta), _ptr(residual), int(relu),
                                  _ptr(y), _ptr(n_dev), n, c, dtype_code(x), _ptr(row_map), _ptr(post_add), _stream()), "bn_apply")
        return y, None
    _check(lib().u3d_bn_apply(_ptr(x), _ptr(mean), _ptr(invstd), _ptr(gamma), _ptr(beta), _ptr(residual), int(relu),
                              _ptr(y), _ptr(n_dev), n, c, dtype_code(x), _ptr(row_map), _ptr(post_add), _stream()), "bn_apply")
    return y


def bn_bwd_stats(dy, y, x, mean, invstd, relu, n_dev, gamma=None, beta=None, row_map=None, want_f32=False):
    n, c = x.shape
    sums = torch.empty((2, c), dtype=torch.float64, device=x.device)
    wsb = int(lib().u3d_bn_stats_workspace(n, c))
    ws = torch.empty(wsb, dtype=torch.uint8, device=x.device)
    s32 = torch.empty((2, c), dtype=torch.float32, device=x.device) if want_f32 else None
    _check(lib().u3d_bn_bwd_stats(_ptr(dy), _ptr(y), _ptr(x), _ptr(mean), _ptr(invstd), _ptr(gamma), _ptr(beta), int(relu), _ptr(n_dev), n, c,
                                  dtype_code(x), _ptr(sums), _ptr(ws), wsb, _ptr(row_map), _ptr(s32), _stream()), "bn_bwd_stats")
    return (sums, s32) if want_f32 else sums


def bn_bwd_apply(dy, y, x, mean, invstd, gamma, sums, relu, n_dev, want_dres, beta=None, row_map=None, want_planes=False):
    n, c = x.shape
    dx = torch.empty_like(x)
    dres = torch.empty_like(x) if want_dres else None
    if want_planes:
        if x.dtype == torch.float32 and x.is_cuda:
            planes = torch.empty((2 * n, c), dtype=torch.bfloat16, device=x.device)
            rc = lib().u3d_bn_bwd_apply_planes(_ptr(dy), _ptr(y), _ptr(x), _ptr(mean), _ptr(invstd), _ptr(gamma), _ptr(beta), _ptr(sums), int(relu),
                                               _ptr(dx), _ptr(dres), _ptr(planes), _ptr(n_dev), n, c, _ptr(row_map), _stream())
            if rc == 0:
                return dx, dres, planes
            if rc != U3D_ERR_UNSUPPORTED:
                _check(rc, "bn_bwd_apply_planes")
        _check(lib().u3d_bn_bwd_apply(_ptr(dy), _ptr(y), _ptr(x), _ptr(mean), _ptr(invstd), _ptr(gamma), _ptr(beta), _ptr(sums), int(relu),
                                      _ptr(dx), _ptr(dres), _ptr(n_dev), n, c, dtype_code(x), _ptr(row_map), _stream()), "bn_bwd_apply")
        return dx, dres, None
    _check(lib().u3d_bn_bwd_apply(_ptr(dy), _ptr(y), _ptr(x), _ptr(mean), _ptr(invstd), _ptr(gamma), _ptr(beta), _ptr(sums), int(relu),
                                  _ptr(dx), _ptr(dres), _ptr(n_dev), n, c, dtype_code(x), _ptr(row_map), _stream()), "bn_bwd_apply")
    return dx, dres


def to_dense(feat, coors, n_dev, batch, dims):
    n, c = feat.shape
    dz, dy, dx = dims
    vol = torch.zeros((batch, dz, dy, dx, c), dtype=feat.dtype, device=feat.device)
    _check(lib().u3d_to_dense(_ptr(feat), _ptr(coors), _ptr(n_dev), n, c, _ptr(vol), dz, dy, dx, dtype_code(feat), _stream()),
           "to_dense")
    return vol.permute(0, 4, 1, 2, 3)


def from_dense(vol_cl, coors, n_dev, n):
    b, dz, dy, dx, c = vol_cl.shape
    feat = torch.empty((n, c), dtype=vol_cl.dtype, device=vol_cl.device)
    _check(lib().u3d_from_dense(_ptr(vol_cl), _ptr(coors), _ptr(n_dev), n, c, _ptr(feat), dz, dy, dx, dtype_code(vol_cl),
                                _stream()), "from_dense")
    return feat


def gather_rows(inp, idx):
    n = idx.shape[0]
    out = torch.empty((n,) + tuple(inp.shape[1:]), dtype=inp.dtype, device=inp.device)
    row_bytes = inp[0].numel() * inp.element_size()
    _check(lib().u3d_gather_rows(_ptr(inp), _ptr(idx), n, row_bytes, _ptr(out), _stream()), "gather_rows")
    return out


def scatter_rows(inp, idx, n_out):
    out = torch.zeros((n_out,) + tuple(inp.shape[1:]), dtype=inp.dtype, device=inp.device)
    row_bytes = inp[0].numel() * inp.element_size()
    _check(lib().u3d_scatter_rows(_ptr(inp), _ptr(idx), idx.shape[0], row_bytes, _ptr(out), _stream()), "scatter_rows")
    return out


FPS_REG_MAX = 20480


def fps_err_buffer(device):
    return torch.zeros(2, dtype=torch.int32, device=device)


def _fps_err_arg(err, max_n, device):
    if max_n <= FPS_REG_MAX:
        return None
    return fps_err_buffer(device) if err is None else err


def fps(base, set_off, set_n, max_n, m, err=None, poll_ticks=0, max_wg=0):
    nsets = set_off.shape[0]
    out = torch.empty((nsets, m), dtype=torch.int32, device=base.device)
    temp, stride = None, 0
    if max_n > FPS_REG_MAX:
        temp = torch.empty((nsets, max_n), dtype=torch.float32, device=base.device)
        stride = max_n
    err = _fps_err_arg(err, max_n, base.device)
    _check(lib().u3d_fps(_ptr(base), _ptr(set_off), _ptr(set_n), nsets, max_n, m, _ptr(out), _ptr(temp), stride, _ptr(err), int(poll_ticks),
                         int(max_wg), _stream()), "fps")
    out._u3d_fps_err = err
    return out


def fps_queries(points, coors, scene_off, voxel_off, batch, max_n, m, err=None, poll_ticks=0, max_wg=0):
    dev = points.device
    F_ = points.shape[1]
    V = coors.shape[0]
    vox = torch.empty((max(V, 1), 3), dtype=torch.float32, device=dev)
    set_off = torch.empty((2 * batch,), dtype=torch.int64, device=dev)
    set_n = torch.empty((2 * batch,), dtype=torch.int32, device=dev)
    _check(lib().u3d_fps_prep(_ptr(coors), V, _ptr(scene_off), _ptr(voxel_off), batch, F_, _ptr(vox), _ptr(set_off), _ptr(set_n), _stream()),
           "fps_prep")
    idx = torch.empty((2 * batch, m), dtype=torch.int32, device=dev)
    temp, stride = None, 0
    if max_n > FPS_REG_MAX:
        temp = torch.empty((2 * batch, max_n), dtype=torch.float32, device=dev)
        stride = max_n
    err = _fps_err_arg(err, max_n, dev)
    _check(lib().u3d_fps2(_ptr(points), _ptr(vox), batch, _ptr(set_off), _ptr(set_n), 2 * batch, max_n, m, _ptr(idx), _ptr(temp), stride,
                          _ptr(err), int(poll_ticks), int(max_wg), _stream()), "fps2")
    idx._u3d_fps_err = err
    out = torch.empty((batch, 2 * m, 3), dtype=torch.float32, device=dev)
    _check(lib().u3d_fps_points(_ptr(points), F_, _ptr(vox), _ptr(idx), _ptr(scene_off), _ptr(voxel_off), batch, m, _ptr(out), _stream()),
           "fps_points")
    return out, idx


def loss_targets(asg, gt, labels, gt_off, ncls):
    L, B, Q = asg.shape
    gd = gt.shape[1]
    dev = asg.device
    a64 = torch.empty((L, B, Q), dtype=torch.int64, device=dev)
    w = torch.empty((L, B, Q), dtype=torch.float32, device=dev)
    tgt = torch.empty((L, B, Q, gd), dtype=torch.float32, device=dev)
    lab = torch.empty((L, B, Q), dtype=torch.int64, device=dev)
    npos = torch.empty((L,), dtype=torch.float32, device=dev)
    _check(lib().u3d_loss_targets(_ptr(asg), _ptr(gt), _ptr(labels), _ptr(gt_off), L, B, Q, gd, ncls, _ptr(a64), _ptr(w), _ptr(tgt), _ptr(lab),
                                  _ptr(npos), _stream()), "loss_targets")
    return a64, w, tgt, lab, npos


def query_embed_fwd(tgt, anchor, fps, rnd, groups):
    B, nq, c = fps.shape[0], anchor.shape[0], tgt.shape[1]
    dev = tgt.device
    qe = torch.empty((B, groups * nq, c + 3), dtype=torch.float32, device=dev)
    q = torch.empty((B, groups * nq, c), dtype=torch.float32, device=dev)
    r = torch.empty((B, groups * nq, 3), dtype=torch.float32, device=dev)
    rs = torch.empty((B, groups * nq, 3), dtype=torch.float32, device=dev)
    _check(lib().u3d_query_embed_fwd(_ptr(tgt), _ptr(anchor), _ptr(fps), _ptr(rnd), B, nq, groups, c, _ptr(qe), _ptr(q), _ptr(r), _ptr(rs),
                                     _stream()), "query_embed_fwd")
    return qe, q, r, rs


def query_embed_bwd(dqe, dq, dr, drs, anchor, B, nq, groups, c, device):
    dt = torch.empty((2 * nq, c), dtype=torch.float32, device=device)
    da = torch.empty((nq, 3), dtype=torch.float32, device=device)
    _check(lib().u3d_query_embed_bwd(_ptr(dqe), _ptr(dq), _ptr(dr), _ptr(drs), _ptr(anchor), B, nq, groups, c, _ptr(dt), _ptr(da), _stream()),
           "query_embed_bwd")
    return dt, da


def match_cost(cls, box, gt, labels, gt_off, gmax, w_cls, w_reg, w_iou, alpha=0.25, gamma=2.0):
    L, B, Q, Ccls = cls.shape
    cost = torch.zeros((L * B, gmax, Q), dtype=torch.float32, device=cls.device)
    _check(lib().u3d_match_cost(_ptr(cls), _ptr(box), _ptr(gt), _ptr(labels), _ptr(gt_off), L, B, Q, Ccls, box.shape[-1], gmax,
                                w_cls, w_reg, w_iou, alpha, gamma, _ptr(cost), _stream()), "match_cost")
    return cost


def lsa(cost, gt_off, L, B, Q, nq, gmax):
    assigned = torch.empty((L, B, Q), dtype=torch.int32, device=cost.device)
    _check(lib().u3d_lsa(_ptr(cost), _ptr(gt_off), L, B, Q, nq, gmax, _ptr(assigned), _stream()), "lsa")
    return assigned


def iou3d_rotated_aligned(a, b):
    n = a.shape[0]
    out = torch.empty((n,), dtype=torch.float32, device=a.device)
    _check(lib().u3d_iou3d_rotated_aligned(_ptr(a), _ptr(b), n, _ptr(out), _stream()), "iou3d_rotated_aligned")
    return out


def trilinear_fwd(value_rows, grid, batch, dims):
    nq, c = grid.shape[1], value_rows.shape[1]
    out = torch.empty((batch, nq, c), dtype=value_rows.dtype, device=value_rows.device)
    _check(lib().u3d_trilinear_fwd(_ptr(value_rows), _ptr(grid), batch, nq, dims[0], dims[1], dims[2], c, _ptr(out),
                                   dtype_code(value_rows), _stream()), "trilinear_fwd")
    return out


def trilinear_bwd(value_rows, grid, dout, batch, dims, want_dvalue=True, want_dgrid=True, dvalue_accum=None):
    nq, c = grid.shape[1], value_rows.shape[1]
    if want_dvalue:
        dvalue = dvalue_accum if dvalue_accum is not None else torch.zeros(value_rows.shape, dtype=torch.float32, device=value_rows.device)
    else:
# ... 942 lines not shown
```

uni3detr_amd/plugin/dense.py:

```python

import numpy as np
import torch
from torch import nn

from .. import native as nv
from .. import sparse as sp
from ..registry import BACKBONES, NECKS


def _conv(cfg, cin, cout, kernel, stride=1, padding=0):
    cfg = dict(cfg)
    t = cfg.pop("type")
    if t != "Conv3d":
        raise NotImplementedError("the HIP dense path implements the Conv3d variant used by every shipped config")
    if cfg.get("bias", True):
        raise NotImplementedError("shipped configs build these convolutions with bias=False")
    return nn.Conv3d(cin, cout, kernel, stride=stride, padding=padding, **cfg)


def _norm(cfg, c):
    cfg = dict(cfg)
    t = cfg.pop("type")
    assert t == "BN3d", "shipped configs use BN3d"
    cfg.pop("requires_grad", None)
    return nn.BatchNorm3d(c, **cfg)


_BRANCH_STREAMS = []
PARALLEL_BRANCHES = True


class Lattice:

    _cache = {}

    @classmethod
    def conv(cls, device, batch, dims_in, ksize, stride, pad):
        key = ("c", str(device), batch, tuple(dims_in), tuple(ksize), tuple(stride), tuple(pad))
        g = cls._cache.get(key)
        if g is None:
            dims_out = tuple((d + 2 * p - k) // s + 1 for d, k, s, p in zip(dims_in, ksize, stride, pad))
            n_in = batch * dims_in[0] * dims_in[1] * dims_in[2]
            n_out = batch * dims_out[0] * dims_out[1] * dims_out[2]
            one = all(k == 1 for k in ksize) and all(s == 1 for s in stride)
            fwd = None if one else nv.dense_nbr_table(batch, dims_out, dims_in, ksize, stride, pad, 0, device)
            bwd = None if one else nv.dense_nbr_table(batch, dims_in, dims_out, ksize, stride, pad, 1, device)
            n_in_dev = torch.tensor([n_in], dtype=torch.int32, device=device)
            n_out_dev = torch.tensor([n_out], dtype=torch.int32, device=device)
            g = (sp.ConvGeom(fwd, bwd, n_in, n_in_dev, n_out, n_out_dev, kind="dense", strided=any(s > 1 for s in stride)), dims_out)
            cls._cache[key] = g
        return g

    @classmethod
    def upsample_index(cls, device, batch, dims_in, s):
        key = ("u", str(device), batch, tuple(dims_in), s)
        v = cls._cache.get(key)
        if v is None:
            D, H, W = dims_in
            b = torch.arange(batch, device=device).view(-1, 1, 1, 1)
            z = torch.arange(D, device=device).view(1, -1, 1, 1)
            y = torch.arange(H * s, device=device).view(1, 1, -1, 1)
            x = torch.arange(W * s, device=device).view(1, 1, 1, -1)
            in_row = ((b * D + z) * H + y // s) * W + x // s
            tap = (y % s) * s + (x % s)
            idx = (in_row * (s * s) + tap).reshape(-1).int().contiguous()
            inv = torch.empty_like(idx)
            inv[idx.long()] = torch.arange(idx.numel(), device=device, dtype=torch.int32)
            v = (idx, inv, (D, H * s, W * s))
            cls._cache[key] = v
        return v


FUSED_LEVEL_SUM = True
FUSED_UPSAMPLE_ORDER = True


class _GatherBijection(torch.autograd.Function):
    @staticmethod
    def forward(ctx, rows, idx, inv):
        ctx.save_for_backward(inv)
        return nv.gather_rows(rows.contiguous(), idx)

    @staticmethod
    def backward(ctx, dout):
        (inv,) = ctx.saved_tensors
        return nv.gather_rows(dout.contiguous(), inv), None, None


def to_rows(x):
    B, C, D, H, W = x.shape
    return x.permute(0, 2, 3, 4, 1).reshape(-1, C), B, (D, H, W)


def to_volume(rows, B, dims):
    return rows.view(B, *dims, rows.shape[1]).permute(0, 4, 1, 2, 3)


def conv_bn_relu(rows, B, dims, conv, bn, post_add=None, fan_token=None):
    ks, st, pd = tuple(conv.kernel_size), tuple(conv.stride), tuple(conv.padding)
    geom, dims_out = Lattice.conv(rows.device, B, dims, ks, st, pd)
    return sp.conv_bn(rows, conv.weight, geom, bn, geom.n_out_dev, None, True, "oidhw", post_add, fan_token=fan_token), dims_out


def deconv_bn_relu(rows, B, dims, deconv, bn, post_add=None):
    s = deconv.stride[1]
    assert tuple(deconv.kernel_size) == (1, s, s) and tuple(deconv.stride) == (1, s, s), "non-overlapping (1,s,s) upsampling only"
    cin, cout = deconv.weight.shape[0], deconv.weight.shape[1]
    n_in = rows.shape[0]
    geom, _ = Lattice.conv(rows.device, B, dims, (1, 1, 1), (1, 1, 1), (0, 0, 0))
    w = deconv.weight.permute(0, 2, 3, 4, 1).reshape(1, 1, 1, cin, s * s * cout)
    y = sp.sparse_conv(rows, w, geom).view(n_in * s * s, cout)
    idx, inv, dims_out = Lattice.upsample_index(rows.device, B, dims, s)
    n_dev = Lattice.conv(rows.device, B, dims_out, (1, 1, 1), (1, 1, 1), (0, 0, 0))[0].n_out_dev
    if FUSED_UPSAMPLE_ORDER:
        return sp.bn_rows(y, bn, n_dev, None, True, row_map=inv, post_add=post_add), dims_out
    y = _GatherBijection.apply(y, idx, inv)
    return sp.bn_rows(y, bn, n_dev, None, True, post_add=post_add), dims_out


FANOUT_FUSION = True


@BACKBONES.register_module()
class SECOND3D(nn.Module):
    def __init__(self, in_channels=128, out_channels=[128, 128, 256], layer_nums=[3, 5, 5], layer_strides=[2, 2, 2],
                 is_cascade=True, norm_cfg=dict(type="BN3d", eps=1e-3, momentum=0.01), conv_cfg=dict(type="Conv3d", bias=False),
                 init_cfg=None, pretrained=None):
        super().__init__()
        assert len(layer_strides) == len(layer_nums) == len(out_channels)
        in_filters = list(in_channels) if isinstance(in_channels, (list, tuple)) else [in_channels, *out_channels[:-1]]
        self.is_cascade = is_cascade
        self.kernel_type = conv_cfg.type if hasattr(conv_cfg, "type") else conv_cfg["type"]
        kernel = tuple(conv_cfg.pop("kernel")) if "kernel" in conv_cfg else (1, 3, 3)
        padding = tuple((k - 1) // 2 for k in kernel)
        blocks = []
        for i, n in enumerate(layer_nums):
            s = layer_strides[i]
            layers = [_conv(conv_cfg, in_filters[i], out_channels[i], kernel, (1, s, s), padding), _norm(norm_cfg, out_channels[i]),
                      nn.ReLU(inplace=True)]
            for _ in range(n):
                layers += [_conv(conv_cfg, out_channels[i], out_channels[i], kernel, 1, padding), _norm(norm_cfg, out_channels[i]),
                           nn.ReLU(inplace=True)]
            blocks.append(nn.Sequential(*layers))
        self.blocks = nn.ModuleList(blocks)

    @staticmethod
    def _run_block(blk, rows, B, dims, fan=None):
        mods = list(blk)
        for j in range(0, len(mods), 3):
            rows, dims = conv_bn_relu(rows, B, dims, mods[j], mods[j + 1], fan_token=fan if j == 0 else None)
        return rows, dims

    def forward(self, x):
        rows, B, dims = to_rows(x)
        outs = []
        if self.is_cascade:
            for blk in self.blocks:
                rows, dims = self._run_block(blk, rows, B, dims)
                outs.append(to_volume(rows, B, dims))
            return tuple(outs)
        if not PARALLEL_BRANCHES or torch.cuda.is_current_stream_capturing():
            fan = sp.FanoutToken(len(self.blocks)) if (FANOUT_FUSION and rows.requires_grad and len(self.blocks) > 1) else None
            seq = [self._run_block(blk, rows, B, dims, fan) for blk in self.blocks]
            return tuple(to_volume(r, B, d) for r, d in seq)
        cur = torch.cuda.current_stream()
        while len(_BRANCH_STREAMS) < len(self.blocks) - 1:
            _BRANCH_STREAMS.append(torch.cuda.Stream())
        results = [None] * len(self.blocks)
        for i in range(len(self.blocks) - 1, 0, -1):
            st = _BRANCH_STREAMS[i - 1]
            st.wait_stream(cur)
            with torch.cuda.stream(st):
                results[i] = self._run_block(self.blocks[i], rows, B, dims)
        results[0] = self._run_block(self.blocks[0], rows, B, dims)
        for i in range(1, len(self.blocks)):
            rows.record_stream(_BRANCH_STREAMS[i - 1])
            cur.wait_stream(_BRANCH_STREAMS[i - 1])
        return tuple(to_volume(r, B, d) for r, d in results)


@NECKS.register_module()
class SECOND3DFPN(nn.Module):
    def __init__(self, in_channels=[128, 128, 256], out_channels=[256, 256, 256], upsample_strides=[1, 2, 4],
                 norm_cfg=dict(type="BN3d", eps=1e-3, momentum=0.01), upsample_cfg=dict(type="deconv3d", bias=False),
                 conv_cfg=dict(type="Conv3d", bias=False), extra_conv=None, use_conv_for_no_stride=False, use_for_distill=False,
                 init_cfg=None):
        super().__init__()
        assert len(out_channels) == len(upsample_strides) == len(in_channels)
        self.in_channels, self.out_channels = in_channels, out_channels
        self.fp16_enabled = False
        if use_for_distill:
            raise NotImplementedError("use_for_distill is not used by any shipped Uni3DETR config")
        assert upsample_cfg["type"] == "deconv3d" and not upsample_cfg.get("bias", True)
        deblocks = []
        for i, oc in enumerate(out_channels):
            s = upsample_strides[i]
            if s > 1 or (s == 1 and not use_conv_for_no_stride):
                up = nn.ConvTranspose3d(in_channels[i], oc, (1, s, s), stride=(1, s, s), bias=False)
            else:
                s2 = int(np.round(1 / s))
                up = _conv(conv_cfg, in_channels[i], oc, (1, s2, s2), (1, s2, s2))
            deblocks.append(nn.Sequential(up, _norm(norm_cfg, oc), nn.ReLU(inplace=True)))
        self.deblocks = nn.ModuleList(deblocks)
        self.extra_conv = extra_conv
        if extra_conv is not None:
            extra = dict(extra_conv)
            self.layer_num = extra.pop("num_conv")
            kernel = tuple(extra.pop("kernel")) if "kernel" in extra else (3, 3, 3)
            if "sep_kernel" in extra:
                raise NotImplementedError("sep_kernel is not used by any shipped Uni3DETR config")
            padding = tuple((k - 1) // 2 for k in kernel)
            layers = []
            for _ in range(self.layer_num):
                layers += [_conv(extra, out_channels[-1], out_channels[-1], kernel, 1, padding), _norm(norm_cfg, out_channels[-1]),
                           nn.ReLU(inplace=True)]
            self.extra_blocks = nn.Sequential(*layers)

    def forward(self, x):
        assert len(x) == len(self.in_channels)
        out, odims, B = None, None, None
        for i, d in enumerate(self.deblocks):
            rows, B, dims = to_rows(x[i])
            fuse = FUSED_LEVEL_SUM and out is not None and rows.is_cuda and out.dtype == rows.dtype
            if isinstance(d[0], nn.ConvTranspose3d):
                r, dd = deconv_bn_relu(rows, B, dims, d[0], d[1], out if fuse else None)
            else:
                r, dd = conv_bn_relu(rows, B, dims, d[0], d[1], out if fuse else None)
            assert odims is None or odims == dd, "FPN levels must land on one lattice"
            out, odims = (r if (out is None or fuse) else out + r), dd
        if self.extra_conv is not None:
            mods = list(self.extra_blocks)
            for j in range(0, len(mods), 3):
                out, odims = conv_bn_relu(out, B, odims, mods[j], mods[j + 1])
        return to_volume(out, B, odims)
```

uni3detr_amd/sparse.py:

```python
import collections
import contextlib
import os

import torch

from . import native as nv
from .shadow import conv_weights, halo_packs

K3, S1, P1 = (3, 3, 3), (1, 1, 1), (1, 1, 1)


class Level:

    def __init__(self, grid, coords, n, n_dev):
        self.grid, self.coords, self.n, self.n_dev = grid, coords, n, n_dev
        self.dims, self.batch = grid.dims, grid.batch
        self._subm = None
        self._halo = None

    def halo(self):
        if self._halo is None:
            h = nv.SubmHalo(self.subm_tables()[0], self.n_dev, self.n) if self.n <= nv.SubmHalo.MAX_ROWS else None
            self._halo = h if (h is not None and h.ok) else False
        return self._halo or None
# ... 341 lines not shown


def _split_input_grad(ctx, r, wc, dys):
    g, kvol, cin, cout = ctx.geom, r.kvol, r.cin, r.cout
    n_out = dys.shape[0] // 2
    w3 = nv.split3_weights(wc, ctx.layout, nmajor=False, cache=ctx.split3)
    if r.split == "narrow":
        return nv.spconv_fwd_split_direct(dys, w3, g.nbr_bwd, g.n_in_dev, g.n_in, cin, tag="spconv_dgrad"), False
    if r.strided_split:
        tid = _split_table(g, "id", n_out, n_out)
        wt3 = w3.view(3, kvol * cin, cout)
        prod = nv.spconv_fwd_split(dys, wt3, tid, g.n_out_dev, n_out, kvol * cin, tag="spconv_dgrad")
        return nv.tap_gather_sum(prod, g.nbr_bwd, g.n_in_dev, g.n_in, cin, kvol), False
    add = _pending_addend(ctx) if SPLIT_FUSED_ADD else None
    if add is not None and not (add.dtype == torch.float32 and add.is_contiguous() and tuple(add.shape) == (g.n_in, cin)):
        add = None
    t3 = _split_table(g, "bwd", g.n_in, n_out)
    return nv.spconv_fwd_split(dys, w3, t3, g.n_in_dev, g.n_in, cin, tag="spconv_dgrad", addend=add), add is not None


def sparse_conv(feats, weight, geom, layout="dhwio", fan_token=None):
    return _SparseConv.apply(feats, weight, geom, layout, False, None, fan_token)


FUSED_CONV_STATS = True


_FOLD = [None]


@contextlib.contextmanager
def fold_scope(table):
    prev = _FOLD[0]
    _FOLD[0] = table
    try:
        yield
    finally:
        _FOLD[0] = prev


def conv_affine(feats, w_folded, shift, geom, relu=True):
    if torch.is_grad_enabled() and (feats.requires_grad or w_folded.requires_grad):
        raise RuntimeError("conv_affine is an inference path: it records no autograd node")
    if feats.dtype != torch.bfloat16 or not feats.is_cuda:
        raise RuntimeError(f"conv_affine needs bf16 device rows, got {feats.dtype} on {feats.device}")
    kvol, cin = w_folded.shape[0], w_folded.shape[2]
    if feats.shape[1] != cin:
        raise ValueError(f"conv_affine: input has {feats.shape[1]} channels, folded weight expects {cin}")
    nv.CALL_KIND = geom.kind
    nbr = geom.nbr_fwd if kvol > 1 else None
    return nv.igemm_fwd_affine(feats.contiguous(), w_folded, nbr, shift, relu, geom.n_out_dev, geom.n_out)


def conv_folded(feats, ent, geom, residual=None, relu=True):
    w_folded, shift, w_packed = ent
    kvol, cout, cin = w_folded.shape
    if torch.is_grad_enabled() and (feats.requires_grad or (residual is not None and residual.requires_grad)):
        raise RuntimeError("a folded conv + BatchNorm pair is an inference path: it records no autograd node")
    if feats.dtype != torch.bfloat16 or not feats.is_cuda:
        raise RuntimeError(f"a folded conv + BatchNorm pair needs bf16 device rows, got {feats.dtype} on {feats.device}")
    if feats.shape[1] != cin:
        raise ValueError(f"folded conv: input has {feats.shape[1]} channels, folded weight expects {cin}")
    if residual is not None and not (residual.dtype == torch.bfloat16 and tuple(residual.shape) == (geom.n_out, cout)):
        raise ValueError("folded conv: the residual must be bf16 rows of the output's shape")
    halo = _halo_of(geom, kvol, cin, cout) if w_packed is not None else None
    if halo is not None:
        nv.CALL_KIND = geom.kind
        return nv.subm_halo_conv_affine(feats.contiguous(), w_packed, halo, shift, relu, None if residual is None else residual.contiguous())
    if nv.direct_serves(cin, cout, kvol) and geom.nbr_fwd is not None:
        nv.CALL_KIND = geom.kind
        return nv.igemm_direct_affine(feats.contiguous(), w_folded, geom.nbr_fwd, shift, relu, geom.n_out_dev, geom.n_out,
                                      None if residual is None else residual.contiguous())
    if residual is None:
        return conv_affine(feats, w_folded, shift, geom, relu)
    return None


def conv_bn(feats, weight, geom, bn, n_dev, residual=None, relu=True, layout="dhwio", post_add=None, res_take=None, res_give=None, fan_token=None):
    if _FOLD[0] is not None:
        ent = _FOLD[0].get(id(bn))
        if ent is not None:
            if len(ent) == 2:
                if bn.training or residual is not None or post_add is not None:
                    raise RuntimeError("a folded conv + BatchNorm pair was called in training mode, or with a residual / level sum")
                return conv_affine(feats, ent[0], ent[1], geom, relu)
            if bn.training or post_add is not None:
                raise RuntimeError("a folded conv + BatchNorm pair of a sparse level was called in training mode, or with a level sum")
            y = conv_folded(feats, ent, geom, residual, relu)
            if y is not None:
                return y
    if FUSED_CONV_STATS and bn.training and feats.is_cuda and (feats.dtype == torch.bfloat16 or _split_serves(feats, feats.shape[1], bn.num_features) == "wide"):
        y, stats = _SparseConv.apply(feats, weight, geom, layout, True, res_take, fan_token)
        if stats.numel():
            tr = getattr(stats, "_u3d_tile_rows", None)
            if tr is None:
                nb = stats.shape[0]
                tr = next((t for t in (128, 256, 192) if (y.shape[0] + t - 1) // t == nb), 0)
            return _BNRows.apply(y, bn.weight, bn.bias, residual, n_dev, bn, relu, True, stats, tr, None, post_add, res_give)
        return _BNRows.apply(y, bn.weight, bn.bias, residual, n_dev, bn, relu, bn.training, None, 0, None, post_add, res_give)
    return bn_rows(sparse_conv(feats, weight, geom, layout, fan_token), bn, n_dev, residual, relu, None, post_add)


class _BNRows(torch.autograd.Function):

    @staticmethod
    def forward(ctx, x, gamma, beta, residual, n_dev, bn, relu, training, stats=None, tile_rows=0, row_map=None, post_add=None, res_token=None):
        n = x.shape[0]
        if training and stats is not None:
            mean, invstd = nv.bn_finalize_partials(stats, tile_rows, n_dev, n, bn.eps, bn.momentum if bn.momentum is not None else 0.1,
                                                   bn.running_mean, bn.running_var, bn.num_batches_tracked)
        elif training:
            mean, invstd = nv.bn_forward_stats(x, n_dev, bn.eps, bn.momentum if bn.momentum is not None else 0.1,
                                               bn.running_mean, bn.running_var, bn.num_batches_tracked)
        else:
            mean = bn.running_mean
            invstd = torch.rsqrt(bn.running_var + bn.eps)
        g32, b32 = gamma.float(), beta.float()
        if post_add is not None:
            assert relu and residual is None and post_add.shape == x.shape and post_add.dtype == x.dtype
            post_add = post_add.contiguous()
        ctx.planes = bool(BN_PLANES and _SPLIT[0] and x.is_cuda and x.dtype == torch.float32 and x.shape[1] % 16 == 0)
        if ctx.planes:
            y, ypl = nv.bn_apply(x, mean, invstd, g32, b32, residual, relu, n_dev, row_map, post_add, want_planes=True)
            _give_planes(y, ypl)
        else:
            y = nv.bn_apply(x, mean, invstd, g32, b32, residual, relu, n_dev, row_map, post_add)
        ctx.remask = bool(relu and residual is None)
        ctx.save_for_backward(x, None if ctx.remask else y, mean, invstd, g32, b32)
        ctx.n_dev, ctx.relu, ctx.training, ctx.has_res = n_dev, relu, training, residual is not None
        ctx.pdtype = gamma.dtype
        ctx.row_map = row_map
        ctx.has_post = post_add is not None
        ctx.res_token = res_token if residual is not None else None
        return y

    @staticmethod
    def backward(ctx, dy):
        x, y, mean, invstd, gamma, beta = ctx.saved_tensors
        dy = dy.contiguous()
        sums, s32 = nv.bn_bwd_stats(dy, y, x, mean, invstd, ctx.relu, ctx.n_dev, gamma, beta, ctx.row_map, want_f32=True)
        use = sums if ctx.training else torch.zeros_like(sums)
        if ctx.planes:
            dx, dres, dpl = nv.bn_bwd_apply(dy, y, x, mean, invstd, gamma, use, ctx.relu, ctx.n_dev, ctx.has_res, beta, ctx.row_map, want_planes=True)
            _give_bwd_planes(dx, dpl)
        else:
            dx, dres = nv.bn_bwd_apply(dy, y, x, mean, invstd, gamma, use, ctx.relu, ctx.n_dev, ctx.has_res, beta, ctx.row_map)
        if ctx.pdtype != torch.float32:
            s32 = s32.to(ctx.pdtype)
        if ctx.res_token is not None and dres is not None:
            ctx.res_token.dres, dres = dres, None
        return dx, s32[1], s32[0], dres, None, None, None, None, None, None, None, (dy if ctx.has_post else None), None


def bn_rows(x, bn, n_dev, residual=None, relu=True, row_map=None, post_add=None):
    return _BNRows.apply(x, bn.weight, bn.bias, residual, n_dev, bn, relu, bn.training, None, 0, row_map, post_add, None)


class _ToDense(torch.autograd.Function):
    @staticmethod
    def forward(ctx, feats, lvl):
        ctx.lvl = lvl
        return nv.to_dense(feats, lvl.coords, lvl.n_dev, lvl.batch, lvl.dims)

    @staticmethod
    def backward(ctx, dvol):
        lvl = ctx.lvl
        cl = dvol.permute(0, 2, 3, 4, 1).contiguous()
        return nv.from_dense(cl, lvl.coords, lvl.n_dev, lvl.n), None


def to_dense(feats, lvl):
    return _ToDense.apply(feats, lvl)


class _PermuteRows(torch.autograd.Function):

    @staticmethod
    def forward(ctx, feats, rank, n_out):
        ctx.save_for_backward(rank)
        return nv.scatter_rows(feats.contiguous(), rank, n_out)

    @staticmethod
    def backward(ctx, dout):
        (rank,) = ctx.saved_tensors
        return nv.gather_rows(dout.contiguous(), rank), None, None


def permute_rows(feats, rank, n_out):
    return _PermuteRows.apply(feats, rank, n_out)
```

Measured before the change: 440.5.

## Batch BatchNorm kernels across parallel backbone branches into multi-tensor launches

Kernel bodies for BN stats, finalize, apply and backward move into a shared include, so they can be instantiated both as single-tensor kernels and as multi-tensor kernels that serve up to four independent tensors in one launch. The dense backbone now runs its branches in lockstep, layer by layer, in bf16 training, and the per-branch BN work goes through these batched launches instead of separate per-branch kernels or per-branch streams. The aim is to cut kernel launch count and fill the GPU better on small branch tensors. The trade-off is that the multi-stream branch parallelism is replaced, which could lose some overlap of the convolutions.

```diff
diff --git a/include/u3d_hip.h b/include/u3d_hip.h
--- a/include/u3d_hip.h
+++ b/include/u3d_hip.h
@@ -206,6 +206,23 @@
 int32_t u3d_bn_bwd_apply_planes(const float* dy, const float* y, const float* x, const float* mean, const float* invstd,
                                 const float* gamma, const float* beta, const double* sums, int32_t relu, float* dx, float* dres,
                                 void* planes, const int32_t* n_dev, int32_t n_cap, int32_t c, const int32_t* row_map, u3d_stream s);
+#define U3D_BN_MULTI_MAX 4
+int32_t u3d_bn_finalize_partials_multi(int32_t count, const double* const* partial, const int32_t* nblocks, const int32_t* rows_per_block,
+                                       const int32_t* const* n_dev, const int32_t* n_cap, const int32_t* c, const float* eps,
+                                       const float* momentum, float* const* running_mean, float* const* running_var,
+                                       int64_t* const* num_batches, float* const* mean, float* const* invstd, u3d_stream s);
+int32_t u3d_bn_apply_multi(int32_t count, const void* const* x, const float* const* mean, const float* const* invstd,
+                           const float* const* gamma, const float* const* beta, const int32_t* relu, void* const* y,
+                           const int32_t* const* n_dev, const int32_t* n_cap, const int32_t* c, u3d_stream s);
+int32_t u3d_bn_bwd_stats_multi(int32_t count, const void* const* dy, const void* const* y, const void* const* x,
+                               const float* const* mean, const float* const* invstd, const float* const* gamma,
+                               const float* const* beta, const int32_t* relu, const int32_t* const* n_dev, const int32_t* n_cap,
+                               const int32_t* c, double* const* sums, void* const* workspace, const int64_t* workspace_bytes,
+                               float* const* sums_f32, u3d_stream s);
+int32_t u3d_bn_bwd_apply_multi(int32_t count, const void* const* dy, const void* const* y, const void* const* x,
+                               const float* const* mean, const float* const* invstd, const float* const* gamma,
+                               const float* const* beta, const double* const* sums, const int32_t* relu, void* const* dx, void* const* dres,
+                               const int32_t* const* n_dev, const int32_t* n_cap, const int32_t* c, u3d_stream s);
 
 int32_t u3d_to_dense(const void* feat, const int32_t* coors, const int32_t* n_dev, int32_t n_cap, int32_t c,
                      void* dense, int32_t dz, int32_t dy, int32_t dx, int32_t dtype, u3d_stream s);
diff --git a/uni3detr_amd/csrc/bn_rows_bodies.inc b/uni3detr_amd/csrc/bn_rows_bodies.inc
--- /dev/null
+++ b/uni3detr_amd/csrc/bn_rows_bodies.inc
@@ -0,0 +1,214 @@
+#ifdef BN_MULTI
+#define BN_BLK blk
+#define BN_NBLK nblk
+#else
+#define BN_BLK blockIdx.x
+#define BN_NBLK gridDim.x
+#endif
+#if BN_BODY == 1
+  constexpr int V = VecOf<T>::N;
+  extern __shared__ __attribute__((aligned(16))) char smem_raw[];
+  double* red = (double*)smem_raw;
+  const int n = min(*n_dev, n_cap);
+  const int cv = c / V;
+  const int cw = cv < 256 ? cv : 256;
+  const int rl = 256 / cw;
+  const int tcol = threadIdx.x % cw, trow = threadIdx.x / cw;
+  const int r0 = BN_BLK * rows_per_block;
+  const int r1 = min(n, r0 + rows_per_block);
+  for (int cb = 0; cb < cv; cb += cw) {
+    const int vc = cb + tcol;
+    float s0[V], s1[V];
+#pragma unroll
+    for (int e = 0; e < V; ++e) { s0[e] = 0.f; s1[e] = 0.f; }
+    const bool active = vc < cv && trow < rl;
+    if (active) {
+      float mu[V], is[V], ga[V], be[V];
+      const bool remask = MODE == 1 && relu && y == nullptr;
+      if (MODE == 1) {
+        load_cols<V>(mean, vc * V, mu);
+        load_cols<V>(invstd, vc * V, is);
+        if (remask) { load_cols<V>(gamma, vc * V, ga); load_cols<V>(beta, vc * V, be); }
+      }
+#pragma unroll 4
+      for (int r = r0 + trow; r < r1; r += rl) {
+        const long long o = (long long)r * c + (long long)vc * V;
+        float xv[V];
+        load_vec<T>(x + o, xv);
+        if (MODE == 0) {
+#pragma unroll
+          for (int e = 0; e < V; ++e) { s0[e] += xv[e]; s1[e] += xv[e] * xv[e]; }
+        } else {
+          float gv[V], yv[V];
+          const long long oy = row_map ? (long long)row_map[r] * c + (long long)vc * V : o;
+          load_vec<T>(dy + oy, gv);
+          if (relu && !remask) load_vec<T>(y + oy, yv);
+#pragma unroll
+          for (int e = 0; e < V; ++e) {
+            float g = gv[e];
+            if (remask) yv[e] = (xv[e] - mu[e]) * is[e] * ga[e] + be[e];
+            if (relu && !(yv[e] > 0.f)) g = 0.f;
+            s0[e] += g;
+            s1[e] += g * ((xv[e] - mu[e]) * is[e]);
+          }
+        }
+      }
+    }
+    const int ncol = cw * V;
+    if (trow < rl) {
+#pragma unroll
+      for (int e = 0; e < V; ++e) {
+        red[(0 * rl + trow) * ncol + tcol * V + e] = (double)s0[e];
+        red[(1 * rl + trow) * ncol + tcol * V + e] = (double)s1[e];
+      }
+    }
+    __syncthreads();
+    const int NP = rl >= 32 ? 8 : 1;
+    if (NP > 1) {
+      double* red2 = red + 2 * rl * ncol;
+      for (int i = threadIdx.x; i < 2 * ncol * NP; i += 256) {
+        const int o = i % (2 * ncol), pp = i / (2 * ncol), which = o / ncol, col = o % ncol;
+        double a = 0.0;
+        for (int j = pp; j < rl; j += NP) a += red[(which * rl + j) * ncol + col];
+        red2[pp * 2 * ncol + o] = a;
+      }
+      __syncthreads();
+      for (int i = threadIdx.x; i < 2 * ncol; i += 256) {
+        const int which = i / ncol, col = i % ncol;
+        if (cb * V + col < c) {
+          double a = 0.0;
+          for (int pp = 0; pp < NP; ++pp) a += red2[pp * 2 * ncol + i];
+          partial[((long long)BN_BLK * 2 + which) * c + cb * V + col] = a;
+        }
+      }
+    } else {
+      for (int i = threadIdx.x; i < 2 * ncol; i += 256) {
+        int which = i / ncol, col = i % ncol;
+        if (cb * V + col < c) {
+          double a = 0.0;
+          for (int j = 0; j < rl; ++j) a += red[(which * rl + j) * ncol + col];
+          partial[((long long)BN_BLK * 2 + which) * c + cb * V + col] = a;
+        }
+      }
+    }
+    __syncthreads();
+  }
+#elif BN_BODY == 2
+  __shared__ double red[FIN_LANES][16];
+  const int n = min(*n_dev, n_cap);
+  int used = rows_per_block > 0 ? (n + rows_per_block - 1) / rows_per_block : nblocks;
+  if (used > nblocks) used = nblocks;
+  const int col0 = BN_BLK * 8;
+  fin_reduce(partial, used, c, col0, red);
+  if (threadIdx.x < 16) {
+    const int which = threadIdx.x >> 3, col = col0 + (threadIdx.x & 7);
+    if (col < c) {
+      const double s = red[0][threadIdx.x];
+      sums[which * c + col] = s;
+      if (sums_f32) sums_f32[which * c + col] = (float)s;
+    }
+  }
+#elif BN_BODY == 3
+  __shared__ double red[FIN_LANES][16];
+  if (BN_BLK == 0 && threadIdx.x == 0 && num_batches) *num_batches += 1;
+  const int n = min(*n_dev, n_cap);
+  int used = rows_per_block > 0 ? (n + rows_per_block - 1) / rows_per_block : nblocks;
+  if (used > nblocks) used = nblocks;
+  const int col0 = BN_BLK * 8;
+  fin_reduce(partial, used, c, col0, red);
+  const int col = col0 + threadIdx.x;
+  if (threadIdx.x >= 8 || col >= c) return;
+  const double s0 = red[0][threadIdx.x], s1 = red[0][8 + threadIdx.x];
+  const double nn = n > 0 ? (double)n : 1.0;
+  const double mu = s0 / nn;
+  double var = s1 / nn - mu * mu;
+  if (var < 0.0) var = 0.0;
+  mean[col] = (float)mu;
+  invstd[col] = (float)(1.0 / sqrt(var + (double)eps));
+  if (running_mean) {
+    const double unbiased = n > 1 ? var * nn / (nn - 1.0) : var;
+    running_mean[col] = (1.f - momentum) * running_mean[col] + momentum * (float)mu;
+    running_var[col] = (1.f - momentum) * running_var[col] + momentum * (float)unbiased;
+  }
+#elif BN_BODY == 4
+  constexpr int V = VecOf<T>::N;
+  static_assert(!PLANES || V == 4, "planes are an f32 feature");
+  const int n = min(*n_dev, n_cap), cv = c / V, rpb = 256 / cv;
+  const int vc = threadIdx.x % cv, rl = threadIdx.x / cv;
+  float mu[V], is[V], ga[V], be[V];
+  load_cols<V>(mean, vc * V, mu); load_cols<V>(invstd, vc * V, is); load_cols<V>(gamma, vc * V, ga); load_cols<V>(beta, vc * V, be);
+  for (int r = BN_BLK * rpb + rl; r < n; r += BN_NBLK * rpb) {
+    const long long o = (long long)r * c + (long long)vc * V;
+    float xv[V], rv[V], out[V];
+    load_vec<T>(x + o, xv);
+    if (res) load_vec<T>(res + o, rv);
+#pragma unroll
+    for (int e = 0; e < V; ++e) {
+      float v = (xv[e] - mu[e]) * is[e] * ga[e] + be[e];
+      if (res) v += rv[e];
+      if (relu) v = v > 0.f ? v : 0.f;
+      out[e] = v;
+    }
+    const long long oy = row_map ? (long long)row_map[r] * c + (long long)vc * V : o;
+    if (post_add) {
+      float pv[V];
+      load_vec<T>(post_add + oy, pv);
+#pragma unroll
+      for (int e = 0; e < V; ++e) out[e] += pv[e];
+    }
+    store_vec<T>(y + oy, out);
+    if constexpr (PLANES) store_planes4(planes + oy, (long long)n_cap * c, out);
+  }
+  if constexpr (PLANES) {
+    const float z[4] = {0.f, 0.f, 0.f, 0.f};
+    for (int r = n + BN_BLK * rpb + rl; r < n_cap; r += BN_NBLK * rpb)
+      store_planes4(planes + (long long)r * c + (long long)vc * V, (long long)n_cap * c, z);
+  }
+#elif BN_BODY == 5
+  constexpr int V = VecOf<T>::N;
+  static_assert(!PLANES || V == 4, "planes are an f32 feature");
+  const int n = min(*n_dev, n_cap), cv = c / V, rpb = 256 / cv;
+  const int vc = threadIdx.x % cv, rl = threadIdx.x / cv;
+  const float inv_n = n > 0 ? 1.f / (float)n : 0.f;
+  const bool remask = relu && y == nullptr;
+  float mu[V], is[V], ga[V], be[V], mg[V], mgx[V];
+  load_cols<V>(mean, vc * V, mu); load_cols<V>(invstd, vc * V, is); load_cols<V>(gamma, vc * V, ga);
+  if (remask) load_cols<V>(beta, vc * V, be);
+  else {
+#pragma unroll
+    for (int e = 0; e < V; ++e) be[e] = 0.f;
+  }
+  load_cols_d<V>(sums, vc * V, inv_n, mg);
+  load_cols_d<V>(sums + c, vc * V, inv_n, mgx);
+#pragma unroll 2
+  for (int r = BN_BLK * rpb + rl; r < n; r += BN_NBLK * rpb) {
+    const long long o = (long long)r * c + (long long)vc * V;
+    float gv[V], xv[V], yv[V], dxv[V];
+    const long long oy = row_map ? (long long)row_map[r] * c + (long long)vc * V : o;
+    load_vec<T>(dy + oy, gv);
+    load_vec<T>(x + o, xv);
+    if (relu && !remask) load_vec<T>(y + oy, yv);
+#pragma unroll
+    for (int e = 0; e < V; ++e) {
+      float g = gv[e];
+      if (remask) yv[e] = (xv[e] - mu[e]) * is[e] * ga[e] + be[e];
+      if (relu && !(yv[e] > 0.f)) g = 0.f;
+      const float xh = (xv[e] - mu[e]) * is[e];
+      dxv[e] = ga[e] * is[e] * (g - mg[e] - xh * mgx[e]);
+      gv[e] = g;
+    }
+    store_vec<T>(dx + o, dxv);
+    if constexpr (PLANES) store_planes4(planes + o, (long long)n_cap * c, dxv);
+    if (dres) store_vec<T>(dres + o, gv);
+  }
+  if constexpr (PLANES) {
+    const float z[4] = {0.f, 0.f, 0.f, 0.f};
+    for (int r = n + BN_BLK * rpb + rl; r < n_cap; r += BN_NBLK * rpb)
+      store_planes4(planes + (long long)r * c + (long long)vc * V, (long long)n_cap * c, z);
+  }
+#else
+#error "BN_BODY names no body"
+#endif
+#undef BN_BLK
+#undef BN_NBLK
+#undef BN_BODY
diff --git a/uni3detr_amd/csrc/rowops.hip b/uni3detr_amd/csrc/rowops.hip
--- a/uni3detr_amd/csrc/rowops.hip
+++ b/uni3detr_amd/csrc/rowops.hip
@@ -60,93 +60,8 @@
                                                        const float* __restrict__ gamma, const float* __restrict__ beta, int relu,
                                                        const int* __restrict__ n_dev, int n_cap, int c, double* __restrict__ partial,
                                                        const int* __restrict__ row_map, int rows_per_block) {
-  constexpr int V = VecOf<T>::N;
-  extern __shared__ __attribute__((aligned(16))) char smem_raw[];
-  double* red = (double*)smem_raw;
-  const int n = min(*n_dev, n_cap);
-  const int cv = c / V;
-  const int cw = cv < 256 ? cv : 256;
-  const int rl = 256 / cw;
-  const int tcol = threadIdx.x % cw, trow = threadIdx.x / cw;
-  const int r0 = blockIdx.x * rows_per_block;
-  const int r1 = min(n, r0 + rows_per_block);
-  for (int cb = 0; cb < cv; cb += cw) {
-    const int vc = cb + tcol;
-    float s0[V], s1[V];
-#pragma unroll
-    for (int e = 0; e < V; ++e) { s0[e] = 0.f; s1[e] = 0.f; }
-    const bool active = vc < cv && trow < rl;
-    if (active) {
-      float mu[V], is[V], ga[V], be[V];
-      const bool remask = MODE == 1 && relu && y == nullptr;
-      if (MODE == 1) {
-        load_cols<V>(mean, vc * V, mu);
-        load_cols<V>(invstd, vc * V, is);
-        if (remask) { load_cols<V>(gamma, vc * V, ga); load_cols<V>(beta, vc * V, be); }
-      }
-#pragma unroll 4
-      for (int r = r0 + trow; r < r1; r += rl) {
-        const long long o = (long long)r * c + (long long)vc * V;
-        float xv[V];
-        load_vec<T>(x + o, xv);
-        if (MODE == 0) {
-#pragma unroll
-          for (int e = 0; e < V; ++e) { s0[e] += xv[e]; s1[e] += xv[e] * xv[e]; }
-        } else {
-          float gv[V], yv[V];
-          const long long oy = row_map ? (long long)row_map[r] * c + (long long)vc * V : o;
-          load_vec<T>(dy + oy, gv);
-          if (relu && !remask) load_vec<T>(y + oy, yv);
-#pragma unroll
-          for (int e = 0; e < V; ++e) {
-            float g = gv[e];
-            if (remask) yv[e] = (xv[e] - mu[e]) * is[e] * ga[e] + be[e];
-            if (relu && !(yv[e] > 0.f)) g = 0.f;
-            s0[e] += g;
-            s1[e] += g * ((xv[e] - mu[e]) * is[e]);
-          }
-        }
-      }
-    }
-    const int ncol = cw * V;
-    if (trow < rl) {
-#pragma unroll
-      for (int e = 0; e < V; ++e) {
-        red[(0 * rl + trow) * ncol + tcol * V + e] = (double)s0[e];
-        red[(1 * rl + trow) * ncol + tcol * V + e] = (double)s1[e];
-      }
-    }
-    __syncthreads();
-    const int NP = rl >= 32 ? 8 : 1;
-    if (NP > 1) {
-      double* red2 = red + 2 * rl * ncol;
-      for (int i = threadIdx.x; i < 2 * ncol * NP; i += 256) {
-        const int o = i % (2 * ncol), pp = i / (2 * ncol), which = o / ncol, col = o % ncol;
-        double a = 0.0;
-        for (int j = pp; j < rl; j += NP) a += red[(which * rl + j) * ncol + col];
-        red2[pp * 2 * ncol + o] = a;
-      }
-      __syncthreads();
-      for (int i = threadIdx.x; i < 2 * ncol; i += 256) {
-        const int which = i / ncol, col = i % ncol;
-        if (cb * V + col < c) {
-          double a = 0.0;
-          for (int pp = 0; pp < NP; ++pp) a += red2[pp * 2 * ncol + i];
-          partial[((long long)blockIdx.x * 2 + which) * c + cb * V + col] = a;
-        }
-      }
-    } else {
-      for (int i = threadIdx.x; i < 2 * ncol; i += 256) {
-        int which = i / ncol, col = i % ncol;
-        if (cb * V + col < c) {
-          double a = 0.0;
-          for (int j = 0; j < rl; ++j) a += red[(which * rl + j) * ncol + col];
-          partial[((long long)blockIdx.x * 2 + which) * c + cb * V + col] = a;
-        }
-      }
-    }
-    __syncthreads();
-  }
+#define BN_BODY 1
+#include "bn_rows_bodies.inc"
 }
 
 template <typename T, int MODE>
@@ -223,20 +138,8 @@
 __global__ __launch_bounds__(FIN_THREADS) void k_col_stats_final(const double* __restrict__ partial, int nblocks, const int* __restrict__ n_dev,
                                                                  int n_cap, int c, double* __restrict__ sums, float* __restrict__ sums_f32,
                                                                  int rows_per_block) {
-  __shared__ double red[FIN_LANES][16];
-  const int n = min(*n_dev, n_cap);
-  int used = rows_per_block > 0 ? (n + rows_per_block - 1) / rows_per_block : nblocks;
-  if (used > nblocks) used = nblocks;
-  const int col0 = blockIdx.x * 8;
-  fin_reduce(partial, used, c, col0, red);
-  if (threadIdx.x < 16) {
-    const int which = threadIdx.x >> 3, col = col0 + (threadIdx.x & 7);
-    if (col < c) {
-      const double s = red[0][threadIdx.x];
-      sums[which * c + col] = s;
-      if (sums_f32) sums_f32[which * c + col] = (float)s;
-    }
-  }
+#define BN_BODY 2
+#include "bn_rows_bodies.inc"
 }
 
 extern "C" int64_t u3d_bn_stats_workspace(int32_t n_cap, int32_t c) {
@@ -512,27 +415,8 @@
                                                                    int n_cap, int c, float eps, float momentum, float* __restrict__ running_mean,
                                                                    float* __restrict__ running_var, long long* __restrict__ num_batches,
                                                                    float* __restrict__ mean, float* __restrict__ invstd) {
-  __shared__ double red[FIN_LANES][16];
-  if (blockIdx.x == 0 && threadIdx.x == 0 && num_batches) *num_batches += 1;
-  const int n = min(*n_dev, n_cap);
-  int used = rows_per_block > 0 ? (n + rows_per_block - 1) / rows_per_block : nblocks;
-  if (used > nblocks) used = nblocks;
-  const int col0 = blockIdx.x * 8;
-  fin_reduce(partial, used, c, col0, red);
-  const int col = col0 + threadIdx.x;
-  if (threadIdx.x >= 8 || col >= c) return;
-  const double s0 = red[0][threadIdx.x], s1 = red[0][8 + threadIdx.x];
-  const double nn = n > 0 ? (double)n : 1.0;
-  const double mu = s0 / nn;
-  double var = s1 / nn - mu * mu;
-  if (var < 0.0) var = 0.0;
-  mean[col] = (float)mu;
-  invstd[col] = (float)(1.0 / sqrt(var + (double)eps));
-  if (running_mean) {
-    const double unbiased = n > 1 ? var * nn / (nn - 1.0) : var;
-    running_mean[col] = (1.f - momentum) * running_mean[col] + momentum * (float)mu;
-    running_var[col] = (1.f - momentum) * running_var[col] + momentum * (float)unbiased;
-  }
+#define BN_BODY 3
+#include "bn_rows_bodies.inc"
 }
 extern "C" int32_t u3d_bn_forward_stats(const void* x, const int32_t* n_dev, int32_t n_cap, int32_t c, int32_t dtype, float eps,
                                         float momentum, float* running_mean, float* running_var, int64_t* num_batches, float* mean,
@@ -597,39 +481,8 @@
                                                       const T* __restrict__ res, int relu, T* __restrict__ y,
                                                       const int* __restrict__ n_dev, int n_cap, int c, const int* __restrict__ row_map,
                                                       const T* __restrict__ post_add, u16* __restrict__ planes = nullptr) {
-  constexpr int V = VecOf<T>::N;
-  static_assert(!PLANES || V == 4, "planes are an f32 feature");
-  const int n = min(*n_dev, n_cap), cv = c / V, rpb = 256 / cv;
-  const int vc = threadIdx.x % cv, rl = threadIdx.x / cv;
-  float mu[V], is[V], ga[V], be[V];
-  load_cols<V>(mean, vc * V, mu); load_cols<V>(invstd, vc * V, is); load_cols<V>(gamma, vc * V, ga); load_cols<V>(beta, vc * V, be);
-  for (int r = blockIdx.x * rpb + rl; r < n; r += gridDim.x * rpb) {
-    const long long o = (long long)r * c + (long long)vc * V;
-    float xv[V], rv[V], out[V];
-    load_vec<T>(x + o, xv);
-    if (res) load_vec<T>(res + o, rv);
-#pragma unroll
-    for (int e = 0; e < V; ++e) {
-      float v = (xv[e] - mu[e]) * is[e] * ga[e] + be[e];
-      if (res) v += rv[e];
-      if (relu) v = v > 0.f ? v : 0.f;
-      out[e] = v;
-    }
-    const long long oy = row_map ? (long long)row_map[r] * c + (long long)vc * V : o;
-    if (post_add) {
-      float pv[V];
-      load_vec<T>(post_add + oy, pv);
-#pragma unroll
-      for (int e = 0; e < V; ++e) out[e] += pv[e];
-    }
-    store_vec<T>(y + oy, out);
-    if constexpr (PLANES) store_planes4(planes + oy, (long long)n_cap * c, out);
-  }
-  if constexpr (PLANES) {
-    const float z[4] = {0.f, 0.f, 0.f, 0.f};
-    for (int r = n + blockIdx.x * rpb + rl; r < n_cap; r += gridDim.x * rpb)
-      store_planes4(planes + (long long)r * c + (long long)vc * V, (long long)n_cap * c, z);
-  }
+#define BN_BODY 4
+#include "bn_rows_bodies.inc"
 }
 
 template <typename T, bool PLANES = false>
@@ -639,47 +492,8 @@
                                                           const double* __restrict__ sums, int relu, T* __restrict__ dx,
                                                           T* __restrict__ dres, const int* __restrict__ n_dev, int n_cap, int c,
                                                           const int* __restrict__ row_map, u16* __restrict__ planes = nullptr) {
-  constexpr int V = VecOf<T>::N;
-  static_assert(!PLANES || V == 4, "planes are an f32 feature");
-  const int n = min(*n_dev, n_cap), cv = c / V, rpb = 256 / cv;
-  const int vc = threadIdx.x % cv, rl = threadIdx.x / cv;
-  const float inv_n = n > 0 ? 1.f / (float)n : 0.f;
-  const bool remask = relu && y == nullptr;
-  float mu[V], is[V], ga[V], be[V], mg[V], mgx[V];
-  load_cols<V>(mean, vc * V, mu); load_cols<V>(invstd, vc * V, is); load_cols<V>(gamma, vc * V, ga);
-  if (remask) load_cols<V>(beta, vc * V, be);
-  else {
-#pragma unroll
-    for (int e = 0; e < V; ++e) be[e] = 0.f;
-  }
-  load_cols_d<V>(sums, vc * V, inv_n, mg);
-  load_cols_d<V>(sums + c, vc * V, inv_n, mgx);
-#pragma unroll 2
-  for (int r = blockIdx.x * rpb + rl; r < n; r += gridDim.x * rpb) {
-    const long long o = (long long)r * c + (long long)vc * V;
-    float gv[V], xv[V], yv[V], dxv[V];
-    const long long oy = row_map ? (long long)row_map[r] * c + (long long)vc * V : o;
-    load_vec<T>(dy + oy, gv);
-    load_vec<T>(x + o, xv);
-    if (relu && !remask) load_vec<T>(y + oy, yv);
-#pragma unroll
-    for (int e = 0; e < V; ++e) {
-      float g = gv[e];
-      if (remask) yv[e] = (xv[e] - mu[e]) * is[e] * ga[e] + be[e];
-      if (relu && !(yv[e] > 0.f)) g = 0.f;
-      const float xh = (xv[e] - mu[e]) * is[e];
-      dxv[e] = ga[e] * is[e] * (g - mg[e] - xh * mgx[e]);
-      gv[e] = g;
-    }
-    store_vec<T>(dx + o, dxv);
-    if constexpr (PLANES) store_planes4(planes + o, (long long)n_cap * c, dxv);
-    if (dres) store_vec<T>(dres + o, gv);
-  }
-  if constexpr (PLANES) {
-    const float z[4] = {0.f, 0.f, 0.f, 0.f};
-    for (int r = n + blockIdx.x * rpb + rl; r < n_cap; r += gridDim.x * rpb)
-      store_planes4(planes + (long long)r * c + (long long)vc * V, (long long)n_cap * c, z);
-  }
+#define BN_BODY 5
+#include "bn_rows_bodies.inc"
 }
 
 static inline bool bn_vec_ok(int c, int v) { return c % v == 0 && (c / v) <= 256 && 256 % (c / v) == 0; }
@@ -739,6 +553,255 @@
   return U3D_OK;
 }
 
+#define BNM U3D_BN_MULTI_MAX
+struct BnMulti {
+  int count, n_cap[BNM], c[BNM], relu[BNM], nblocks[BNM], rows_per_block[BNM];
+  float eps[BNM], momentum[BNM];
+  const int* n_dev[BNM];
+  const void *x[BNM], *dy[BNM], *y[BNM];
+  void *out[BNM], *dres[BNM];
+  float *mean[BNM], *invstd[BNM];
+  const float *gamma[BNM], *beta[BNM];
+  const double* partial[BNM];
+  void* workspace[BNM];
+  double* sums[BNM];
+  float *sums_f32[BNM], *running_mean[BNM], *running_var[BNM];
+  long long* num_batches[BNM];
+};
+#undef BNM
+struct BnMultiGrid { int first[U3D_BN_MULTI_MAX + 1]; int slot[U3D_BN_MULTI_MAX]; };
+__device__ __forceinline__ int bn_multi_slot(const BnMultiGrid& g, unsigned b, unsigned& local) {
+  int p = 0;
+#pragma unroll
+  for (int i = 1; i < U3D_BN_MULTI_MAX; ++i) if (b >= (unsigned)g.first[i]) p = i;
+  local = b - (unsigned)g.first[p];
+  return g.slot[p];
+}
+static int bn_multi_grid(const int* blocks, int count, BnMultiGrid* g) {
+  int order[U3D_BN_MULTI_MAX];
+  for (int i = 0; i < count; ++i) order[i] = i;
+  for (int i = 1; i < count; ++i)
+    for (int j = i; j > 0 && blocks[order[j]] > blocks[order[j - 1]]; --j) { const int t = order[j]; order[j] = order[j - 1]; order[j - 1] = t; }
+  int total = 0;
+  for (int p = 0; p < U3D_BN_MULTI_MAX; ++p) {
+    g->first[p] = total;
+    g->slot[p] = p < count ? order[p] : 0;
+    if (p < count) total += blocks[order[p]];
+  }
+  g->first[U3D_BN_MULTI_MAX] = total;
+  return total;
+}
+
+#define BN_MULTI
+__global__ __launch_bounds__(256) void k_col_stats_multi(BnMulti d, BnMultiGrid g) {
+  typedef u16 T;
+  constexpr int MODE = 1;
+  unsigned blk;
+  const int t = bn_multi_slot(g, blockIdx.x, blk);
+  const T* __restrict__ x = (const T*)d.x[t];
+  const T* __restrict__ dy = (const T*)d.dy[t];
+  const T* __restrict__ y = (const T*)d.y[t];
+  const float* __restrict__ mean = d.mean[t];
+  const float* __restrict__ invstd = d.invstd[t];
+  const float* __restrict__ gamma = d.gamma[t];
+  const float* __restrict__ beta = d.beta[t];
+  const int relu = d.relu[t], n_cap = d.n_cap[t], c = d.c[t], rows_per_block = d.rows_per_block[t];
+  const int* __restrict__ n_dev = d.n_dev[t];
+  double* __restrict__ partial = (double*)d.workspace[t];
+  const int* __restrict__ row_map = nullptr;
+#define BN_BODY 1
+#include "bn_rows_bodies.inc"
+}
+__global__ __launch_bounds__(FIN_THREADS) void k_col_stats_final_multi(BnMulti d, BnMultiGrid g) {
+  unsigned blk;
+  const int t = bn_multi_slot(g, blockIdx.x, blk);
+  const double* __restrict__ partial = (const double*)d.workspace[t];
+  const int nblocks = d.nblocks[t], n_cap = d.n_cap[t], c = d.c[t], rows_per_block = d.rows_per_block[t];
+  const int* __restrict__ n_dev = d.n_dev[t];
+  double* __restrict__ sums = d.sums[t];
+  float* __restrict__ sums_f32 = d.sums_f32[t];
+#define BN_BODY 2
+#include "bn_rows_bodies.inc"
+}
+__global__ __launch_bounds__(FIN_THREADS) void k_bn_final_finalize_multi(BnMulti d, BnMultiGrid g) {
+  unsigned blk;
+  const int t = bn_multi_slot(g, blockIdx.x, blk);
+  const double* __restrict__ partial = d.partial[t];
+  const int nblocks = d.nblocks[t], n_cap = d.n_cap[t], c = d.c[t], rows_per_block = d.rows_per_block[t];
+  const int* __restrict__ n_dev = d.n_dev[t];
+  const float eps = d.eps[t], momentum = d.momentum[t];
+  float* __restrict__ running_mean = d.running_mean[t];
+  float* __restrict__ running_var = d.running_var[t];
+  long long* __restrict__ num_batches = (long long*)d.num_batches[t];
+  float* __restrict__ mean = d.mean[t];
+  float* __restrict__ invstd = d.invstd[t];
+#define BN_BODY 3
+#include "bn_rows_bodies.inc"
+}
+__global__ __launch_bounds__(256) void k_bn_apply_multi(BnMulti d, BnMultiGrid g) {
+  typedef u16 T;
+  constexpr bool PLANES = false;
+  unsigned blk;
+  const int t = bn_multi_slot(g, blockIdx.x, blk);
+  const unsigned nblk = (unsigned)d.nblocks[t];
+  const T* __restrict__ x = (const T*)d.x[t];
+  const float* __restrict__ mean = d.mean[t];
+  const float* __restrict__ invstd = d.invstd[t];
+  const float* __restrict__ gamma = d.gamma[t];
+  const float* __restrict__ beta = d.beta[t];
+  const T* __restrict__ res = nullptr;
+  const int relu = d.relu[t], n_cap = d.n_cap[t], c = d.c[t];
+  T* __restrict__ y = (T*)d.out[t];
+  const int* __restrict__ n_dev = d.n_dev[t];
+  const int* __restrict__ row_map = nullptr;
+  const T* __restrict__ post_add = nullptr;
+  u16* __restrict__ planes = nullptr;
+#define BN_BODY 4
+#include "bn_rows_bodies.inc"
+}
+__global__ __launch_bounds__(256) void k_bn_bwd_apply_multi(BnMulti d, BnMultiGrid g) {
+  typedef u16 T;
+  constexpr bool PLANES = false;
+  unsigned blk;
+  const int t = bn_multi_slot(g, blockIdx.x, blk);
+  const unsigned nblk = (unsigned)d.nblocks[t];
+  const T* __restrict__ dy = (const T*)d.dy[t];
+  const T* __restrict__ y = (const T*)d.y[t];
+  const T* __restrict__ x = (const T*)d.x[t];
+  const float* __restrict__ mean = d.mean[t];
+  const float* __restrict__ invstd = d.invstd[t];
+  const float* __restrict__ gamma = d.gamma[t];
+  const float* __restrict__ beta = d.beta[t];
+  const double* __restrict__ sums = d.sums[t];
+  const int relu = d.relu[t], n_cap = d.n_cap[t], c = d.c[t];
+  T* __restrict__ dx = (T*)d.out[t];
+  T* __restrict__ dres = (T*)d.dres[t];
+  const int* __restrict__ n_dev = d.n_dev[t];
+  const int* __restrict__ row_map = nullptr;
+  u16* __restrict__ planes = nullptr;
+#define BN_BODY 5
+#include "bn_rows_bodies.inc"
+}
+#undef BN_MULTI
+
+#define BNM_TAKE(F, a)                                                                     \
+  do {                                                                                     \
+    if (a) for (int i_ = 0; i_ < count; ++i_) d.F[i_] = (std::remove_reference_t<decltype(d.F[0])>)(a)[i_]; \
+  } while (0)
+static int bn_multi_check(const BnMulti& d) {
+  for (int i = 0; i < d.count; ++i) {
+    U3D_REQUIRE(d.n_dev[i] && d.mean[i] && d.invstd[i] && d.c[i] > 0, U3D_ERR_ARG);
+    if (!bn_vec_ok(d.c[i], 8) || !(al16(d.mean[i]) && al16(d.invstd[i]) && al16(d.gamma[i]) && al16(d.beta[i]) && al16(d.sums[i])))
+      return U3D_ERR_UNSUPPORTED;
+  }
+  return U3D_OK;
+}
+#define BNM_BEGIN()                                                                                       \
+  U3D_REQUIRE(count >= 1 && n_dev && n_cap && c && mean && invstd, U3D_ERR_ARG);                          \
+  if (count > U3D_BN_MULTI_MAX) return U3D_ERR_UNSUPPORTED;                                               \
+  BnMulti d = {};                                                                                         \
+  d.count = count;                                                                                        \
+  BNM_TAKE(n_dev, n_dev); BNM_TAKE(n_cap, n_cap); BNM_TAKE(c, c); BNM_TAKE(mean, mean); BNM_TAKE(invstd, invstd)
+#define BNM_CHECK()                          \
+  do {                                       \
+    const int rc_ = bn_multi_check(d);       \
+    if (rc_ != U3D_OK) return rc_;           \
+  } while (0)
+
+extern "C" int32_t u3d_bn_finalize_partials_multi(int32_t count, const double* const* partial, const int32_t* nblocks,
+                                                  const int32_t* rows_per_block, const int32_t* const* n_dev, const int32_t* n_cap,
+                                                  const int32_t* c, const float* eps, const float* momentum, float* const* running_mean,
+                                                  float* const* running_var, int64_t* const* num_batches, float* const* mean,
+                                                  float* const* invstd, u3d_stream s) {
+  BNM_BEGIN();
+  U3D_REQUIRE(partial && nblocks && rows_per_block && eps && momentum, U3D_ERR_ARG);
+  BNM_TAKE(partial, partial); BNM_TAKE(nblocks, nblocks); BNM_TAKE(rows_per_block, rows_per_block); BNM_TAKE(eps, eps);
+  BNM_TAKE(momentum, momentum); BNM_TAKE(running_mean, running_mean); BNM_TAKE(running_var, running_var); BNM_TAKE(num_batches, num_batches);
+  BNM_CHECK();
+  int fin[U3D_BN_MULTI_MAX];
+  for (int i = 0; i < count; ++i) {
+    U3D_REQUIRE(d.partial[i] && d.nblocks[i] >= 0 && d.rows_per_block[i] >= 0 && (!d.running_mean[i] || d.running_var[i]), U3D_ERR_ARG);
+    fin[i] = u3d_cdiv(d.c[i], 8);
+  }
+  BnMultiGrid g;
+  const int nb = bn_multi_grid(fin, count, &g);
+  hipLaunchKernelGGL(k_bn_final_finalize_multi, dim3(nb), dim3(FIN_THREADS), 0, s, d, g);
+  U3D_CHECK_LAUNCH();
+  return U3D_OK;
+}
+static int bn_multi_apply_grid(BnMulti* d, BnMultiGrid* g) {
+  int blocks[U3D_BN_MULTI_MAX];
+  for (int i = 0; i < d->count; ++i) d->nblocks[i] = blocks[i] = d->n_cap[i] > 0 ? bn_vec_grid(d->n_cap[i], d->c[i], 8) : 0;
+  return bn_multi_grid(blocks, d->count, g);
+}
+extern "C" int32_t u3d_bn_apply_multi(int32_t count, const void* const* x, const float* const* mean, const float* const* invstd,
+                                      const float* const* gamma, const float* const* beta, const int32_t* relu, void* const* y,
+                                      const int32_t* const* n_dev, const int32_t* n_cap, const int32_t* c, u3d_stream s) {
+  BNM_BEGIN();
+  U3D_REQUIRE(x && gamma && beta && relu && y, U3D_ERR_ARG);
+  BNM_TAKE(x, x); BNM_TAKE(gamma, gamma); BNM_TAKE(beta, beta); BNM_TAKE(relu, relu); BNM_TAKE(out, y);
+  BNM_CHECK();
+  for (int i = 0; i < count; ++i) U3D_REQUIRE(d.x[i] && d.gamma[i] && d.beta[i] && d.out[i], U3D_ERR_ARG);
+  BnMultiGrid g;
+  const int nb = bn_multi_apply_grid(&d, &g);
+  if (nb <= 0) return U3D_OK;
+  hipLaunchKernelGGL(k_bn_apply_multi, dim3(nb), dim3(256), 0, s, d, g);
+  U3D_CHECK_LAUNCH();
+  return U3D_OK;
+}
+extern "C" int32_t u3d_bn_bwd_stats_multi(int32_t count, const void* const* dy, const void* const* y, const void* const* x,
+                                          const float* const* mean, const float* const* invstd, const float* const* gamma,
+                                          const float* const* beta, const int32_t* relu, const int32_t* const* n_dev,
+                                          const int32_t* n_cap, const int32_t* c, double* const* sums, void* const* workspace,
+                                          const int64_t* workspace_bytes, float* const* sums_f32, u3d_stream s) {
+  BNM_BEGIN();
+  U3D_REQUIRE(dy && x && relu && sums && workspace && workspace_bytes, U3D_ERR_ARG);
+  BNM_TAKE(dy, dy); BNM_TAKE(y, y); BNM_TAKE(x, x); BNM_TAKE(gamma, gamma); BNM_TAKE(beta, beta); BNM_TAKE(relu, relu);
+  BNM_TAKE(sums, sums); BNM_TAKE(workspace, workspace); BNM_TAKE(sums_f32, sums_f32);
+  BNM_CHECK();
+  int blocks[U3D_BN_MULTI_MAX], fin[U3D_BN_MULTI_MAX];
+  size_t lds = 0;
+  for (int i = 0; i < count; ++i) {
+    const int nc = d.n_cap[i], ch = d.c[i];
+    U3D_REQUIRE(d.x[i] && d.dy[i] && d.sums[i] && (!d.relu[i] || d.y[i] || (d.gamma[i] && d.beta[i])), U3D_ERR_ARG);
+    U3D_REQUIRE(nc <= 0 || (d.workspace[i] && workspace_bytes[i] >= u3d_bn_stats_workspace(nc, ch)), U3D_ERR_WORKSPACE);
+    d.rows_per_block[i] = st_rows_per_block(nc, ch);
+    d.nblocks[i] = blocks[i] = nc > 0 ? u3d_cdiv(nc, d.rows_per_block[i]) : 0;
+    fin[i] = u3d_cdiv(ch, 8);
+    const int cw = ch / 8, rl = 256 / cw;
+    const size_t l = (size_t)2 * (rl + (rl >= 32 ? 8 : 0)) * cw * 8 * sizeof(double);
+    if (l > lds) lds = l;
+  }
+  BnMultiGrid g;
+  const int nb = bn_multi_grid(blocks, count, &g);
+  if (nb > 0) hipLaunchKernelGGL(k_col_stats_multi, dim3(nb), dim3(256), lds, s, d, g);
+  hipLaunchKernelGGL(k_col_stats_final_multi, dim3(bn_multi_grid(fin, count, &g)), dim3(FIN_THREADS), 0, s, d, g);
+  U3D_CHECK_LAUNCH();
+  return U3D_OK;
+}
+extern "C" int32_t u3d_bn_bwd_apply_multi(int32_t count, const void* const* dy, const void* const* y, const void* const* x,
+                                          const float* const* mean, const float* const* invstd, const float* const* gamma,
+                                          const float* const* beta, const double* const* sums, const int32_t* relu, void* const* dx,
+                                          void* const* dres, const int32_t* const* n_dev, const int32_t* n_cap, const int32_t* c,
+                                          u3d_stream s) {
+  BNM_BEGIN();
+  U3D_REQUIRE(dy && x && gamma && sums && relu && dx, U3D_ERR_ARG);
+  BNM_TAKE(dy, dy); BNM_TAKE(y, y); BNM_TAKE(x, x); BNM_TAKE(gamma, gamma); BNM_TAKE(beta, beta); BNM_TAKE(sums, sums); BNM_TAKE(relu, relu);
+  BNM_TAKE(out, dx); BNM_TAKE(dres, dres);
+  BNM_CHECK();
+  for (int i = 0; i < count; ++i)
+    U3D_REQUIRE(d.dy[i] && d.x[i] && d.gamma[i] && d.sums[i] && d.out[i] && (!d.relu[i] || d.y[i] || d.beta[i]), U3D_ERR_ARG);
+  BnMultiGrid g;
+  const int nb = bn_multi_apply_grid(&d, &g);
+  if (nb <= 0) return U3D_OK;
+  hipLaunchKernelGGL(k_bn_bwd_apply_multi, dim3(nb), dim3(256), 0, s, d, g);
+  U3D_CHECK_LAUNCH();
+  return U3D_OK;
+}
+#undef BNM_BEGIN
+#undef BNM_CHECK
+#undef BNM_TAKE
+
 extern "C" int32_t u3d_bn_apply_planes(const float* x, const float* mean, const float* invstd, const float* gamma, const float* beta,
                                        const float* residual, int32_t relu, float* y, void* planes, const int32_t* n_dev, int32_t n_cap,
                                        int32_t c, const int32_t* row_map, const float* post_add, u3d_stream s) {
diff --git a/uni3detr_amd/native.py b/uni3detr_amd/native.py
--- a/uni3detr_amd/native.py
+++ b/uni3detr_amd/native.py
@@ -922,6 +922,89 @@
     _check(lib().u3d_bn_bwd_apply(_ptr(dy), _ptr(y), _ptr(x), _ptr(mean), _ptr(invstd), _ptr(gamma), _ptr(beta), _ptr(sums), int(relu),
                                   _ptr(dx), _ptr(dres), _ptr(n_dev), n, c, dtype_code(x), _ptr(row_map), _stream()), "bn_bwd_apply")
     return dx, dres
+
+
+BN_MULTI_MAX = _K["U3D_BN_MULTI_MAX"]
+
+
+class _BnMultiArgs:
+
+    def __init__(self, xs, n_devs):
+        self.k = len(xs)
+        self.ok = 1 <= self.k <= BN_MULTI_MAX and all(x.dtype == torch.bfloat16 and x.is_cuda for x in xs)
+        self.n_dev = self.ptrs(n_devs)
+        self.n_cap, self.c = self.ints([x.shape[0] for x in xs]), self.ints([x.shape[1] for x in xs])
+
+    def ptrs(self, tensors):
+        arr = (C.c_void_p * self.k)()
+        for i, t in enumerate(tensors):
+            if t is not None:
+                assert t.is_cuda and t.is_contiguous(), "device-contiguous tensor required"
+                arr[i] = t.data_ptr()
+        return arr
+
+    def ints(self, vals):
+        return (C.c_int32 * self.k)(*(int(v) for v in vals))
+
+    def longs(self, vals):
+        return (C.c_int64 * self.k)(*(int(v) for v in vals))
+
+    def floats(self, vals):
+        return (C.c_float * self.k)(*vals)
+
+    @staticmethod
+    def done(rc, what):
+        if rc == U3D_ERR_UNSUPPORTED:
+            return False
+        _check(rc, what)
+        return True
+
+
+def bn_finalize_partials_multi(xs, stats, tile_rows, n_devs, eps, momentum, running_means, running_vars, num_batches):
+    a = _BnMultiArgs(xs, n_devs)
+    if not a.ok:
+        return None
+    dev = xs[0].device
+    means = [torch.empty((x.shape[1],), dtype=torch.float32, device=dev) for x in xs]
+    invstds = [torch.empty((x.shape[1],), dtype=torch.float32, device=dev) for x in xs]
+    rc = lib().u3d_bn_finalize_partials_multi(a.k, a.ptrs(stats), a.ints(s.shape[0] for s in stats), a.ints(tile_rows), a.n_dev, a.n_cap, a.c,
+                                              a.floats(eps), a.floats(momentum), a.ptrs(running_means), a.ptrs(running_vars),
+                                              a.ptrs(num_batches), a.ptrs(means), a.ptrs(invstds), _stream())
+    return (means, invstds) if a.done(rc, "bn_finalize_partials_multi") else None
+
+
+def bn_apply_multi(xs, means, invstds, gammas, betas, relus, n_devs):
+    a = _BnMultiArgs(xs, n_devs)
+    if not a.ok:
+        return None
+    ys = [torch.empty_like(x) for x in xs]
+    rc = lib().u3d_bn_apply_multi(a.k, a.ptrs(xs), a.ptrs(means), a.ptrs(invstds), a.ptrs(gammas), a.ptrs(betas), a.ints(relus), a.ptrs(ys),
+                                  a.n_dev, a.n_cap, a.c, _stream())
+    return ys if a.done(rc, "bn_apply_multi") else None
+
+
+def bn_bwd_stats_multi(dys, ys, xs, means, invstds, relus, n_devs, gammas, betas):
+    a = _BnMultiArgs(xs, n_devs)
+    if not a.ok:
+        return None
+    dev = xs[0].device
+    sums = [torch.empty((2, x.shape[1]), dtype=torch.float64, device=dev) for x in xs]
+    s32 = [torch.empty((2, x.shape[1]), dtype=torch.float32, device=dev) for x in xs]
+    wsb = [int(lib().u3d_bn_stats_workspace(x.shape[0], x.shape[1])) for x in xs]
+    ws = [torch.empty(b, dtype=torch.uint8, device=dev) for b in wsb]
+    rc = lib().u3d_bn_bwd_stats_multi(a.k, a.ptrs(dys), a.ptrs(ys), a.ptrs(xs), a.ptrs(means), a.ptrs(invstds), a.ptrs(gammas), a.ptrs(betas),
+                                      a.ints(relus), a.n_dev, a.n_cap, a.c, a.ptrs(sums), a.ptrs(ws), a.longs(wsb), a.ptrs(s32), _stream())
+    return (sums, s32) if a.done(rc, "bn_bwd_stats_multi") else None
+
+
+def bn_bwd_apply_multi(dys, ys, xs, means, invstds, gammas, sums, relus, n_devs, betas):
+    a = _BnMultiArgs(xs, n_devs)
+    if not a.ok:
+        return None
+    dxs = [torch.empty_like(x) for x in xs]
+    rc = lib().u3d_bn_bwd_apply_multi(a.k, a.ptrs(dys), a.ptrs(ys), a.ptrs(xs), a.ptrs(means), a.ptrs(invstds), a.ptrs(gammas), a.ptrs(betas),
+                                      a.ptrs(sums), a.ints(relus), a.ptrs(dxs), None, a.n_dev, a.n_cap, a.c, _stream())
+    return dxs if a.done(rc, "bn_bwd_apply_multi") else None
 
 
 def to_dense(feat, coors, n_dev, batch, dims):
diff --git a/uni3detr_amd/plugin/dense.py b/uni3detr_amd/plugin/dense.py
--- a/uni3detr_amd/plugin/dense.py
+++ b/uni3detr_amd/plugin/dense.py
@@ -119,6 +119,7 @@
 
 
 FANOUT_FUSION = True
+BRANCH_BN_BATCH = True
 
 
 @BACKBONES.register_module()
@@ -151,6 +152,19 @@
             rows, dims = conv_bn_relu(rows, B, dims, mods[j], mods[j + 1], fan_token=fan if j == 0 else None)
         return rows, dims
 
+    def _run_lockstep(self, rows, B, dims, fan, small_first=False):
+        mods = [list(blk) for blk in self.blocks]
+        cur = [(rows, dims)] * len(mods)
+        for j in range(0, max(len(m) for m in mods), 3):
+            live = [i for i, m in enumerate(mods) if j < len(m)][::-1 if small_first else 1]
+            convs = [mods[i][j] for i in live]
+            gd = [Lattice.conv(rows.device, B, cur[i][1], tuple(c.kernel_size), tuple(c.stride), tuple(c.padding)) for i, c in zip(live, convs)]
+            ys = sp.conv_bn_multi([cur[i][0] for i in live], [c.weight for c in convs], [g for g, _ in gd], [mods[i][j + 1] for i in live],
+                                  [g.n_out_dev for g, _ in gd], True, "oidhw", [fan if j == 0 else None] * len(live))
+            for i, y, (_, dims_out) in zip(live, ys, gd):
+                cur[i] = (y, dims_out)
+        return cur
+
     def forward(self, x):
         rows, B, dims = to_rows(x)
         outs = []
@@ -159,10 +173,14 @@
                 rows, dims = self._run_block(blk, rows, B, dims)
                 outs.append(to_volume(rows, B, dims))
             return tuple(outs)
-        if not PARALLEL_BRANCHES or torch.cuda.is_current_stream_capturing():
+        batch = BRANCH_BN_BATCH and self.training and rows.is_cuda and rows.dtype == torch.bfloat16 and len(self.blocks) > 1
+        one_stream = not PARALLEL_BRANCHES or torch.cuda.is_current_stream_capturing()
+        if one_stream:
             fan = sp.FanoutToken(len(self.blocks)) if (FANOUT_FUSION and rows.requires_grad and len(self.blocks) > 1) else None
-            seq = [self._run_block(blk, rows, B, dims, fan) for blk in self.blocks]
+            seq = self._run_lockstep(rows, B, dims, fan) if batch else [self._run_block(blk, rows, B, dims, fan) for blk in self.blocks]
             return tuple(to_volume(r, B, d) for r, d in seq)
+        if batch:
+            return tuple(to_volume(r, B, d) for r, d in self._run_lockstep(rows, B, dims, None, small_first=True))
         cur = torch.cuda.current_stream()
         while len(_BRANCH_STREAMS) < len(self.blocks) - 1:
             _BRANCH_STREAMS.append(torch.cuda.Stream())
diff --git a/uni3detr_amd/sparse.py b/uni3detr_amd/sparse.py
--- a/uni3detr_amd/sparse.py
+++ b/uni3detr_amd/sparse.py
@@ -517,6 +517,76 @@
         return dx, s32[1], s32[0], dres, None, None, None, None, None, None, None, (dy if ctx.has_post else None), None
 
 
+def _momentum(bn):
+    return bn.momentum if bn.momentum is not None else 0.1
+
+
+class _BNRowsMulti(torch.autograd.Function):
+
+    @staticmethod
+    def forward(ctx, k, n_devs, bns, relu, stats, tile_rows, *tensors):
+        xs, gammas, betas = tensors[:k], tensors[k:2 * k], tensors[2 * k:]
+        r = nv.bn_finalize_partials_multi(xs, stats, tile_rows, n_devs, [bn.eps for bn in bns], [_momentum(bn) for bn in bns],
+                                          [bn.running_mean for bn in bns], [bn.running_var for bn in bns], [bn.num_batches_tracked for bn in bns])
+        if r is None:
+            r = tuple(zip(*(nv.bn_finalize_partials(st, tr, nd, x.shape[0], bn.eps, _momentum(bn), bn.running_mean, bn.running_var,
+                                                    bn.num_batches_tracked) for x, st, tr, nd, bn in zip(xs, stats, tile_rows, n_devs, bns))))
+        means, invstds = r
+        g32, b32 = [g.float() for g in gammas], [b.float() for b in betas]
+        relus = [relu] * k
+        ys = nv.bn_apply_multi(xs, means, invstds, g32, b32, relus, n_devs)
+        if ys is None:
+            ys = [nv.bn_apply(x, m, i, g, b, None, relu, nd) for x, m, i, g, b, nd in zip(xs, means, invstds, g32, b32, n_devs)]
+        ctx.save_for_backward(*xs, *means, *invstds, *g32, *b32)
+        ctx.k, ctx.n_devs, ctx.relu, ctx.pdtypes = k, n_devs, relu, [g.dtype for g in gammas]
+        return tuple(ys)
+
+    @staticmethod
+    def backward(ctx, *dys):
+        k, relu, n_devs = ctx.k, ctx.relu, ctx.n_devs
+        t = ctx.saved_tensors
+        xs, means, invstds, gammas, betas = (t[i * k:(i + 1) * k] for i in range(5))
+        dys = [dy.contiguous() for dy in dys]
+        none, relus = [None] * k, [relu] * k
+        r = nv.bn_bwd_stats_multi(dys, none, xs, means, invstds, relus, n_devs, gammas, betas)
+        if r is None:
+            r = tuple(zip(*(nv.bn_bwd_stats(dy, None, x, m, i, relu, nd, g, b, None, want_f32=True)
+                            for dy, x, m, i, nd, g, b in zip(dys, xs, means, invstds, n_devs, gammas, betas))))
+        sums, s32 = r
+        dxs = nv.bn_bwd_apply_multi(dys, none, xs, means, invstds, gammas, sums, relus, n_devs, betas)
+        if dxs is None:
+            dxs = [nv.bn_bwd_apply(dy, None, x, m, i, g, s, relu, nd, False, b)[0]
+                   for dy, x, m, i, g, s, nd, b in zip(dys, xs, means, invstds, gammas, sums, n_devs, betas)]
+        s32 = [s if dt == torch.float32 else s.to(dt) for s, dt in zip(s32, ctx.pdtypes)]
+        return (None,) * 6 + tuple(dxs) + tuple(s[1] for s in s32) + tuple(s[0] for s in s32)
+
+
+def _tile_rows(y, stats):
+    tr = getattr(stats, "_u3d_tile_rows", None)
+    if tr is None:
+        nb = stats.shape[0]
+        tr = next((t for t in (128, 256, 192) if (y.shape[0] + t - 1) // t == nb), 0)
+    return tr
+
+
+def conv_bn_multi(feats, weights, geoms, bns, n_devs, relu=True, layout="dhwio", fan_tokens=None):
+    k = len(feats)
+    fans = fan_tokens if fan_tokens is not None else [None] * k
+
+    def vec_ok(c):
+        return c % 8 == 0 and 256 % (c // 8) == 0
+
+    if not (FUSED_CONV_STATS and _FOLD[0] is None and 2 <= k <= nv.BN_MULTI_MAX
+            and all(bn.training and f.is_cuda and f.dtype == torch.bfloat16 and vec_ok(bn.num_features) for f, bn in zip(feats, bns))):
+        return [conv_bn(f, w, g, bn, nd, None, relu, layout, fan_token=fan) for f, w, g, bn, nd, fan in zip(feats, weights, geoms, bns, n_devs, fans)]
+    ys, stats = zip(*(_SparseConv.apply(f, w, g, layout, True, None, fan) for f, w, g, fan in zip(feats, weights, geoms, fans)))
+    if all(st.numel() for st in stats):
+        return list(_BNRowsMulti.apply(k, list(n_devs), list(bns), relu, list(stats), [_tile_rows(y, st) for y, st in zip(ys, stats)],
+                                       *ys, *(bn.weight for bn in bns), *(bn.bias for bn in bns)))
+    return [_BNRows.apply(y, bn.weight, bn.bias, None, nd, bn, relu, True, st if st.numel() else None, _tile_rows(y, st) if st.numel() else 0,
+                          None, None, None) for y, st, bn, nd in zip(ys, stats, bns, n_devs)]
+
+
 def bn_rows(x, bn, n_dev, residual=None, relu=True, row_map=None, post_add=None):
     return _BNRows.apply(x, bn.weight, bn.bias, residual, n_dev, bn, relu, bn.training, None, 0, row_map, post_add, None)
 
```

Result: no change. 444.0, median of 6 (+0.8%).
